# Twinklebear/tray_rust

Measured on NVIDIA H100. Metric: Mrays/s (primary+secondary), higher is better.
Workload: dtype f32

## Files before the change

tray_rust_b200/csrc/trb_api.cu:

```cuda
#include <chrono>
#include <dlfcn.h>
#include <nccl.h>
#include <cstdio>
#include <cstdlib>
#include <memory>
#include <thread>
#include <cub/device/device_radix_sort.cuh>
#include "trb_host.h"
#include "trb_kernels.cuh"

using namespace trbh;

namespace {

thread_local std::string g_error;
unsigned long long g_launches = 0;
trb_status fail(trb_status s, const std::string& msg) { g_error = msg; return s; }

#define CU(call)                                                                                                   \
    do {                                                                                                           \
        cudaError_t e_ = (call);                                                                                   \
        if (e_ != cudaSuccess) return fail(e_ == cudaErrorMemoryAllocation ? TRB_OOM : TRB_CUDA,                   \
                                           std::string(#call) + ": " + cudaGetErrorString(e_));                    \
    } while (0)
// ... 76 lines not shown
        for (int k = 0; k < 3; ++k) if (!(in[c].bmin[k] >= in[p].bmin[k] && in[c].bmax[k] <= in[p].bmax[k])) return false;
        return true;
    };
    if (in.empty()) { root_ref = QUAD_EMPTY_HOST; return true; }
    if (is_leaf(0)) { root_ref = leaf_ref(0); return ok; }
    std::vector<uint32_t> quad_of(in.size(), 0xffffffffu), order, todo{0};
    while (!todo.empty()) {
        const uint32_t p = todo.back(); todo.pop_back();
        quad_of[p] = (uint32_t)order.size(); order.push_back(p);
        uint32_t kids[4]; int nk = 0;
        for (uint32_t c : {p + 1, in[p].a}) {
            if (is_leaf(c)) continue;
            const uint32_t g0 = c + 1, g1 = in[c].a;
            if (inside(g0, c) && inside(g1, c)) { if (!is_leaf(g0)) kids[nk++] = g0; if (!is_leaf(g1)) kids[nk++] = g1; }
            else kids[nk++] = c;
        }
        for (int k = nk; k-- > 0;) todo.push_back(kids[k]);
    }
    if (order.size() >= (1u << 30)) return false;
    out.resize(order.size());
    auto slot = [&](trb::DQuad& q, int k, uint32_t node, bool empty) {
        if (empty) { q.q[2 * k] = make_float4(0.f, 0.f, 0.f, bits_f(0xffffffffu)); q.q[2 * k + 1] = make_float4(0.f, 0.f, 0.f, 0.f); return; }
        const uint32_t ref = is_leaf(node) ? leaf_ref(node) : (trb::REF_INTERIOR | quad_of[node]);
        q.q[2 * k] = make_float4(in[node].bmin[0], in[node].bmin[1], in[node].bmin[2], bits_f(ref));
        q.q[2 * k + 1] = make_float4(in[node].bmax[0], in[node].bmax[1], in[node].bmax[2], 0.f);
    };
    for (size_t qi = 0; qi < order.size(); ++qi) {
        const uint32_t p = order[qi];
        trb::DQuad& q = out[qi];
        uint32_t axes[2] = {0, 0};
        int h = 0;
        for (uint32_t c : {p + 1, in[p].a}) {
            bool split = false;
            if (!is_leaf(c)) { const uint32_t g0 = c + 1, g1 = in[c].a; split = inside(g0, c) && inside(g1, c); }
            if (split) { slot(q, 2 * h, c + 1, false); slot(q, 2 * h + 1, in[c].a, false); axes[h] = in[c].b & 3u; }
            else { slot(q, 2 * h, c, false); slot(q, 2 * h + 1, 0, true); }
            ++h;
        }
        q.q[1].w = bits_f((in[p].b & 3u) | axes[0] << 2 | axes[1] << 4);
    }
    root_ref = trb::REF_INTERIOR | quad_of[0];
    return ok;
}

}

namespace {
struct Tuning {
    int refill = 8;
    unsigned trace_grid = 0;
    uint32_t sched = 6;
    int quads = 0;
    int exact_box = 0;
    int pipe = 36;
    int film_v2 = 1;
    int sort = 0;
    int sort_bits = 5;
    int sort_min_round = 1;
    int shade_anim_occ = 4;
    int frame_device = 1;
    int anim_table = 2;
    int shade_split = -1;
    int shade_sort = 1;
    int shade_kind = 1;
    uint64_t pass_paths = 1ull << 24;
};
int env_int(const char* name, int dflt) { const char* v = getenv(name); return v ? (int)strtol(v, nullptr, 0) : dflt; }
void tuning_from_env(Tuning& t) {
    t.refill = env_int("TRB_REFILL", t.refill); t.trace_grid = (unsigned)env_int("TRB_TRACE_GRID", (int)t.trace_grid);
    t.sched = (uint32_t)env_int("TRB_TRACE_SCHED", (int)t.sched); t.quads = env_int("TRB_TRACE_QUADS", t.quads); t.pipe = env_int("TRB_TRACE_PIPE", t.pipe);
    t.film_v2 = env_int("TRB_FILM_V2", t.film_v2); t.sort = env_int("TRB_SORT", t.sort); t.sort_bits = env_int("TRB_SORT_BITS", t.sort_bits);
    t.sort_min_round = env_int("TRB_SORT_MIN_ROUND", t.sort_min_round); t.shade_split = env_int("TRB_SHADE_SPLIT", t.shade_split); t.anim_table = env_int("TRB_ANIM_TABLE", t.anim_table); t.frame_device = env_int("TRB_FRAME_DEVICE", t.frame_device);
    if (getenv("TRB_PASS_PATHS")) t.pass_paths = strtoull(getenv("TRB_PASS_PATHS"), nullptr, 0);
}

}

struct BlockList {
    uint32_t key[5];
    std::vector<uint32_t> host;
    uint2* dev = nullptr;
};

struct trb_scene {
    int device = 0;
    int sm_count = 0;
    Tuning tune;
    trb_film film{};
    trb_integrator integrator{};
    std::vector<trb_camera> cameras;
    std::vector<trb_instance> instances;
    std::vector<trb_spline> splines;
    std::vector<trb_keyframe> keyframes;
    std::vector<float> knots;
    std::vector<trb_color_key> color_keys;
    std::vector<float> fov_floats;
    std::vector<trb_material> materials;
    std::vector<HostMesh> meshes;
    uint32_t spp_pow2 = 1;
    uint32_t n_anim = 0;
    bool frame_set = false; uint32_t last_frame = 0; float last_start = 0, last_end = 0;
    uint32_t material_kinds = 0;
    bool mixed_materials = false;
    bool anim_emission = false;
    uint32_t* d_anim_instances = nullptr;
    int active_camera = -1;
    float shutter_open = 0, shutter_close = 0;
    std::vector<Xf> world;
    std::vector<trb_bvh_node> tlas_nodes;
    std::vector<uint32_t> tlas_order;
    float table[256];
    DeviceArena arena;
    trb::DScene ds{};
    trb::DInstance* d_instances = nullptr;
    trb::DPair* d_tlas = nullptr;
    trb::DQuad* d_tlas_quads = nullptr;
    trb::DBvh* d_tlas_hdr = nullptr;
    uint32_t* d_tlas_order = nullptr;
    size_t tlas_capacity = 0;
    trb_bvh_node* d_tlas_nodes = nullptr;
    float* d_bounds = nullptr;
    float* d_build_f = nullptr;
    uint32_t* d_build_u = nullptr;
    uint32_t* d_build_counts = nullptr;
    uint32_t tlas_n_nodes = 0;
    bool instances_static_uploaded = false, host_frame_stale = false;
    std::vector<BlockList> block_lists;
    uint32_t* d_counter = nullptr;
    int* d_error = nullptr;
    trb::DStats* d_stats = nullptr;
    float4* d_film = nullptr;
    float* h_film_staging = nullptr;
    cudaEvent_t ev0 = nullptr, ev1 = nullptr;
    bool frame_ready = false;
    trb::WfState wf{};
    size_t wf_capacity = 0;
    std::vector<void*> wf_allocs;
    std::vector<std::pair<cudaEvent_t, cudaEvent_t>> trace_events;
    std::vector<std::pair<cudaEvent_t, cudaEvent_t>> event_pool;
    uint4* d_ad_state = nullptr;
    uint2* d_ad_list[2] = {nullptr, nullptr};
    uint32_t* d_ad_index[2] = {nullptr, nullptr};
    uint32_t* d_ad_flags = nullptr;
    uint32_t* d_ad_count = nullptr;
    uint32_t* d_ad_spp = nullptr;
    void* d_film_scratch = nullptr;
    size_t film_scratch_bytes = 0;
    ~trb_scene() {
        for (void* p : {(void*)d_ad_state, (void*)d_ad_list[0], (void*)d_ad_list[1], (void*)d_ad_index[0], (void*)d_ad_index[1], (void*)d_ad_flags,
                        (void*)d_ad_count, (void*)d_ad_spp, d_film_scratch}) if (p) cudaFree(p);
        for (auto& b : block_lists) cudaFree(b.dev);
        for (void* p : wf_allocs) cudaFree(p);
        for (auto& e : trace_events) { cudaEventDestroy(e.first); cudaEventDestroy(e.second); }
        for (auto& e : event_pool) { cudaEventDestroy(e.first); cudaEventDestroy(e.second); }
        if (h_film_staging) cudaFreeHost(h_film_staging);
        if (ev0) cudaEventDestroy(ev0);
        if (ev1) cudaEventDestroy(ev1);
    }
};

namespace {

Box3 shape_bounds(const trb_scene& s, const trb_instance& in) {
    Box3 b;
    switch (in.shape) {
        case TRB_SHAPE_SPHERE: for (int i = 0; i < 3; ++i) { b.lo[i] = -in.p0; b.hi[i] = in.p0; } break;
        case TRB_SHAPE_DISK: b.lo[0] = b.lo[1] = -in.p0; b.hi[0] = b.hi[1] = in.p0; b.lo[2] = -0.1f; b.hi[2] = 0.1f; break;
        case TRB_SHAPE_RECT: { const float hw = in.p0 / 2.0f, hh = in.p1 / 2.0f; b.lo[0] = -hw; b.lo[1] = -hh; b.hi[0] = hw; b.hi[1] = hh; b.lo[2] = b.hi[2] = 0.0f; break; }
        case TRB_SHAPE_MESH: b = s.meshes[in.mesh].bounds; break;
        default: for (int i = 0; i < 3; ++i) b.lo[i] = b.hi[i] = 0.0f;
    }
    return b;
}

trb_status validate(const trb_scene_desc* d) {
    if (!d) return fail(TRB_INVALID_ARG, "null scene description");
    if (d->abi_version != TRB_ABI_VERSION) return fail(TRB_INVALID_ARG, "trb_scene_desc.abi_version mismatch");
    if (d->film.width == 0 || d->film.height == 0 || d->film.width % 8 || d->film.height % 8)
        return fail(TRB_INVALID_ARG, "Image not evenly divided by blocks of (8, 8)");
    if (d->film.frames == 0) return fail(TRB_INVALID_ARG, "film.frames must be >= 1");
    if (d->n_instances == 0) return fail(TRB_INVALID_ARG, "Aborting: the scene does not have any objects!");
    if (d->n_cameras == 0) return fail(TRB_INVALID_ARG, "Error: A camera is required!");
    if (d->integrator.type > TRB_INTEGRATOR_NORMALS_DEBUG) return fail(TRB_INVALID_ARG, "Unrecognized integrator type");
    if (d->integrator.type == TRB_INTEGRATOR_PATH && d->integrator.max_depth > 57u) return fail(TRB_UNSUPPORTED, "max_depth > 57");
    if (d->integrator.type == TRB_INTEGRATOR_WHITTED && d->integrator.max_depth > 24u) return fail(TRB_UNSUPPORTED, "whitted max_depth > 24 (device recursion stack)");
    if (!(d->film.filter_w > 0.0f && d->film.filter_h > 0.0f)) return fail(TRB_INVALID_ARG, "filter width/height must be positive");
    if (floorf(d->film.filter_w / 0.5f) > 8.0f || floorf(d->film.filter_h / 0.5f) > 8.0f) return fail(TRB_UNSUPPORTED, "filter wider than 4 pixels");
    bool light = false;
    for (uint32_t i = 0; i < d->n_instances; ++i) {
        const trb_instance& in = d->instances[i];
        if (in.kind > TRB_INST_EMITTER_POINT || in.shape > TRB_SHAPE_MESH) return fail(TRB_INVALID_ARG, "unknown instance kind/shape");
        if (in.kind != TRB_INST_EMITTER_POINT && in.shape == TRB_SHAPE_NONE) return fail(TRB_INVALID_ARG, "instance without geometry");
        if (in.kind == TRB_INST_EMITTER_AREA && in.shape == TRB_SHAPE_MESH)
            return fail(TRB_INVALID_ARG, "Geometry of type 'mesh' is not sampleable and can't be used for area light geometry");
        if (in.shape == TRB_SHAPE_MESH && in.mesh >= d->n_meshes) return fail(TRB_INVALID_ARG, "mesh index out of range");
        if (in.kind != TRB_INST_EMITTER_POINT && in.material >= d->n_materials) return fail(TRB_INVALID_ARG, "material index out of range");
        if ((uint64_t)in.spline_first + in.n_splines > d->n_splines) return fail(TRB_INVALID_ARG, "spline range out of bounds");
        if (in.kind != TRB_INST_RECEIVER) {
            light = true;
            if (in.n_emission == 0 || (uint64_t)in.emission_first + in.n_emission > d->n_color_keys) return fail(TRB_INVALID_ARG, "An emission color is required for emitters");
        }
    }
    for (uint32_t k = 0; k < d->n_splines; ++k) {
        const trb_spline& sp = d->splines[k];
        if (sp.n_ctrl == 0 || (uint64_t)sp.ctrl_first + sp.n_ctrl > d->n_keyframes) return fail(TRB_INVALID_ARG, "spline control points out of bounds");
        if (sp.n_ctrl > 1) {
            if ((uint64_t)sp.knot_first + sp.n_knots > d->n_knots) return fail(TRB_INVALID_ARG, "spline knots out of bounds");
            if (sp.n_ctrl <= sp.degree) return fail(TRB_INVALID_ARG, "Too few control points for curve");
            if ((uint64_t)sp.n_knots != (uint64_t)sp.n_ctrl + sp.degree + 1) return fail(TRB_INVALID_ARG, "Invalid B-spline: knots.len() != control_points.len() + degree + 1");
            if (sp.degree > (uint32_t)trbh::kMaxSplineDegree) return fail(TRB_UNSUPPORTED, "B-spline degree above 5");
            for (uint32_t i = 0; i < sp.n_knots; ++i) if (d->knots[sp.knot_first + i] != d->knots[sp.knot_first + i]) return fail(TRB_INVALID_ARG, "NaN knot in B-spline");
        }
    }
    if (!light) return fail(TRB_INVALID_ARG, "At least one light is required");
    for (uint32_t i = 0; i < d->n_cameras; ++i) {
        const trb_camera& c = d->cameras[i];
        if (c.n_fov_ctrl) {
            if ((uint64_t)c.fov_ctrl_first + c.n_fov_ctrl > d->n_fov_floats || (uint64_t)c.fov_knot_first + c.n_fov_knots > d->n_fov_floats) return fail(TRB_INVALID_ARG, "fov spline out of bounds");
            if (c.n_fov_ctrl <= c.fov_degree) return fail(TRB_INVALID_ARG, "Too few control points for curve");
            if ((uint64_t)c.n_fov_knots != (uint64_t)c.n_fov_ctrl + c.fov_degree + 1) return fail(TRB_INVALID_ARG, "Invalid B-spline: knots.len() != control_points.len() + degree + 1");
            for (uint32_t i = 0; i < c.n_fov_knots; ++i) if (d->fov_floats[c.fov_knot_first + i] != d->fov_floats[c.fov_knot_first + i]) return fail(TRB_INVALID_ARG, "NaN knot in B-spline");
            if (c.fov_degree > (uint32_t)trbh::kMaxSplineDegree) return fail(TRB_UNSUPPORTED, "B-spline degree above 5");
        }
        if ((uint64_t)c.spline_first + c.n_splines > d->n_splines) return fail(TRB_INVALID_ARG, "camera spline range out of bounds");
    }
    for (uint32_t i = 0; i < d->n_materials; ++i) {
        if (d->materials[i].type > TRB_MAT_MERL) return fail(TRB_INVALID_ARG, "unrecognized material type");
        if (d->materials[i].type == TRB_MAT_MERL && d->materials[i].merl >= d->n_merl) return fail(TRB_INVALID_ARG, "merl table index out of range");
        for (int k = 0; k < 4; ++k) if (d->materials[i].tex[k] > d->n_textures) return fail(TRB_INVALID_ARG, "texture index out of range");
    }
    uint64_t texels = 0;
    for (uint32_t i = 0; i < d->n_textures; ++i)
        if (d->textures[i].n_images == 0 || (uint64_t)d->textures[i].first_image + d->textures[i].n_images > d->n_images) return fail(TRB_INVALID_ARG, "texture image range out of bounds");
    for (uint32_t i = 0; i < d->n_images; ++i) {
        if (d->images[i].width == 0 || d->images[i].height == 0 || !d->images[i].rgba8) return fail(TRB_INVALID_ARG, "empty image");
        texels += (uint64_t)d->images[i].width * d->images[i].height;
    }
    if (texels >= (1ull << 32)) return fail(TRB_UNSUPPORTED, "more than 2^32 texels of image textures");
    for (uint32_t i = 0; i < d->n_meshes; ++i) {
        const trb_mesh& m = d->meshes[i];
        if (m.n_tris == 0 || m.n_verts == 0) return fail(TRB_INVALID_ARG, "empty mesh");
        if (!m.positions || !m.normals || !m.texcoords || !m.indices) return fail(TRB_INVALID_ARG, "Normals and texture coordinates are required!");
        for (size_t k = 0; k < 3 * (size_t)m.n_tris; ++k) if (m.indices[k] >= m.n_verts) return fail(TRB_INVALID_ARG, "mesh index out of range");
    }
    return TRB_OK;
}

trb_status ensure_blocks(trb_scene* s, const trb_render_cfg* cfg, const uint2** d_blocks, uint32_t* n_blocks) {
    if (cfg->shard_count > 1 && cfg->shard_index >= cfg->shard_count) return fail(TRB_INVALID_ARG, "shard_index must be < shard_count");
    const uint32_t key[5] = {cfg->block_start, cfg->block_count, cfg->shard_index, cfg->shard_count, cfg->shard_chunk};
    for (const BlockList& b : s->block_lists)
        if (std::memcmp(b.key, key, sizeof key) == 0) { *d_blocks = b.dev; *n_blocks = (uint32_t)(b.host.size() / 2); return TRB_OK; }
    if (s->block_lists.size() >= 16) {
        CU(cudaDeviceSynchronize());
        for (BlockList& b : s->block_lists) cudaFree(b.dev);
        s->block_lists.clear();
    }
    BlockList bl;
    std::memcpy(bl.key, key, sizeof key);
    bl.host = morton_blocks(s->film.width, s->film.height, cfg->block_start, cfg->block_count, cfg->shard_index, cfg->shard_count, cfg->shard_chunk);
    const size_t n = bl.host.size() / 2;
    CU(cudaMalloc(reinterpret_cast<void**>(&bl.dev), std::max<size_t>(1, n) * sizeof(uint2)));
    if (n) { cudaError_t e = cudaMemcpy(bl.dev, bl.host.data(), n * sizeof(uint2), cudaMemcpyHostToDevice); if (e != cudaSuccess) { cudaFree(bl.dev); CU(e); } }
    s->block_lists.push_back(std::move(bl));
    *d_blocks = s->block_lists.back().dev; *n_blocks = (uint32_t)n;
    return TRB_OK;
}

trb_status resolve_samples(const trb_scene* s, const trb_render_cfg* cfg, uint32_t& spp, uint32_t& first, uint32_t& count) {
    if (cfg->spp > (1u << 31)) return fail(TRB_INVALID_ARG, "spp too large");
    spp = cfg->spp ? pow2_ceil(cfg->spp) : s->spp_pow2;
    first = cfg->sample_first;
    if (first > spp) return fail(TRB_INVALID_ARG, "sample_first exceeds spp");
    count = cfg->sample_count ? cfg->sample_count : spp - first;
    if ((uint64_t)first + count > spp) return fail(TRB_INVALID_ARG, "sample range exceeds spp");
    return TRB_OK;
}

template <bool STATS, int MODE, bool ANIM>
trb_status launch_render_t(trb_scene* s, const trb::RenderParams& rp, uint32_t flags, cudaStream_t st) {
    const int T = 9 + 2 * std::max(s->ds.fpw_x, s->ds.fpw_y);
    const size_t smem = (size_t)T * T * sizeof(float4);
    int per_sm = 0;
    CU(cudaOccupancyMaxActiveBlocksPerMultiprocessor(&per_sm, trb::k_render<STATS, MODE, ANIM>, trb::RENDER_THREADS, smem));
    const uint32_t grid = std::max(1u, std::min<uint32_t>(rp.n_blocks, (uint32_t)(std::max(1, per_sm) * s->sm_count)));
    trb::k_render<STATS, MODE, ANIM><<<grid, trb::RENDER_THREADS, smem, st>>>(s->ds, rp, flags);
    g_launches++;
    CU(cudaGetLastError());
    return TRB_OK;
}
trb_status ensure_wavefront(trb_scene* s, size_t n_paths) {
    if (n_paths <= s->wf_capacity) return TRB_OK;
    CU(cudaDeviceSynchronize());
    for (void* p : s->wf_allocs) cudaFree(p);
    s->wf_allocs.clear(); s->wf_capacity = 0;
    const size_t cap = n_paths;
    cudaError_t err = cudaSuccess;
    auto grab = [&](size_t bytes, void** out) {
        if (err != cudaSuccess) return;
        err = cudaMalloc(out, bytes);
        if (err == cudaSuccess) s->wf_allocs.push_back(*out);
    };
    trb::WfState& w = s->wf;
    float4** f4[] = {&w.org, &w.cont, &w.shadow, &w.mis, &w.a, &w.b, &w.tprev, &w.thr, &w.illum, &w.ng, &w.rad, &w.f_p, &w.f_n, &w.f_t, &w.f_b};
    for (float4** q : f4) grab(cap * sizeof(float4), reinterpret_cast<void**>(q));
    grab(cap * sizeof(uint4), reinterpret_cast<void**>(&w.hit));
    uint32_t** u1[] = {&w.q_active[0], &w.q_active[1], &w.q_ending[0], &w.q_ending[1], &w.q_cont, &w.q_shadow, &w.q_mis};
    for (uint32_t** q : u1) grab(cap * sizeof(uint32_t), reinterpret_cast<void**>(q));
    grab(cap * trb::WF_MID_BUCKETS * sizeof(uint32_t), reinterpret_cast<void**>(&w.q_mid));
    grab(64 * trb::WF_CNT * sizeof(uint32_t), reinterpret_cast<void**>(&w.counters));
    const size_t max_bins = (size_t)3 * (8u << (3 * trb::WF_SORT_MAX_BITS));
    uint32_t** u3[] = {&w.q_sorted, &w.sort_key, &w.sort_rank};
    for (uint32_t** q : u3) grab(3 * cap * sizeof(uint32_t), reinterpret_cast<void**>(q));
    grab(max_bins * sizeof(uint32_t), reinterpret_cast<void**>(&w.sort_hist));
    grab(max_bins * sizeof(uint32_t), reinterpret_cast<void**>(&w.sort_offs));
    grab(64 * 8 * sizeof(uint32_t), reinterpret_cast<void**>(&w.bounds));
    w.xf_tab = nullptr; w.n_anim = s->n_anim;
    if (s->n_anim) grab(cap * (size_t)s->n_anim * 32 * sizeof(float), reinterpret_cast<void**>(&w.xf_tab));
    if (err == cudaSuccess) err = cudaMemset(w.sort_hist, 0, max_bins * sizeof(uint32_t));
    if (err != cudaSuccess) {
        for (void* p : s->wf_allocs) cudaFree(p);
        s->wf_allocs.clear();
        cudaGetLastError();
        return fail(err == cudaErrorMemoryAllocation ? TRB_OOM : TRB_CUDA, std::string("wavefront state: ") + cudaGetErrorString(err));
    }
    s->wf_capacity = cap;
    return TRB_OK;
}

void launch_anim_table(trb_scene* s, trb::WfState& wf, size_t n_paths, bool adapt, cudaStream_t st) {
    if (!(s->ds.has_anim && wf.xf_tab && s->tune.anim_table)) { wf.xf_tab = nullptr; return; }
    const size_t items = n_paths * wf.n_anim;
    const uint32_t nu = s->ds.n_uniq_splines;
    if (s->tune.anim_table >= 2 && nu > 0 && nu <= 256) {
        const uint32_t per_iter = std::max(1u, std::min(32u, 128u / nu));
        const size_t smem = (size_t)per_iter * nu * 32 * sizeof(float);
        const unsigned grid = (unsigned)std::min<size_t>((n_paths + per_iter - 1) / per_iter, (size_t)s->sm_count * 16);
        if (adapt) trb::k_wf_anim_table2<true><<<grid, 128, smem, st>>>(s->ds, wf, per_iter);
        else trb::k_wf_anim_table2<<<grid, 128, smem, st>>>(s->ds, wf, per_iter);
    } else {
        const unsigned grid = (unsigned)std::min<size_t>((items + 127) / 128, (size_t)s->sm_count * 16);
        if (adapt) trb::k_wf_anim_table<true><<<grid, 128, 0, st>>>(s->ds, wf);
        else trb::k_wf_anim_table<<<grid, 128, 0, st>>>(s->ds, wf);
    }
    g_launches++;
}

void launch_query_trace(trb_scene* s, const trb::RenderParams& rp, const trb::WfState& wf, uint32_t tflags, bool stats, const uint32_t* q_sorted,
                        cudaStream_t st) {
    const Tuning& tu = s->tune;
    const bool anim = s->ds.has_anim != 0;
    const unsigned resident = stats ? 4u : (anim ? 8u : 9u);
    const unsigned tgrid = (unsigned)s->sm_count * (tu.trace_grid ? tu.trace_grid : 2u * resident);
    const uint32_t sched = std::max(1u, tu.sched);
    if (anim) {
        if (stats) trb::k_wf_trace<true, 4, 16, true, true, false, 97><<<tgrid, 128, 0, st>>>(s->ds, rp, wf, 0, tflags, tu.refill, sched, q_sorted);
        else trb::k_wf_trace<false, 8, 12, true, true, false, 97><<<tgrid, 128, 0, st>>>(s->ds, rp, wf, 0, tflags, tu.refill, sched, q_sorted);
    } else if (stats) trb::k_wf_trace<true, 4, 16, false, true, false, 97><<<tgrid, 128, 0, st>>>(s->ds, rp, wf, 0, tflags, tu.refill, sched, q_sorted);
    else trb::k_wf_trace<false, 9, 12, false, true, false, 97><<<tgrid, 128, 0, st>>>(s->ds, rp, wf, 0, tflags, tu.refill, sched, q_sorted);
}

template <int MODE>
void launch_shade(trb_scene* s, const trb::RenderParams& rp, const trb::WfState& wf, uint32_t round, cudaStream_t st) {
    const Tuning& tu = s->tune;
    const bool anim = s->ds.has_anim != 0;
    const unsigned shade_grid = (unsigned)s->sm_count * 4;
    constexpr int MB = MODE == 2 ? 2 : 0;
    const bool split_auto = s->mixed_materials || (tu.shade_sort && tu.shade_kind && s->material_kinds == (1u << TRB_MAT_MATTE));
    if (tu.shade_split > 0 || (tu.shade_split < 0 && split_auto)) {
        const uint32_t all = 0xffu, own = (tu.shade_sort && tu.shade_kind) ? (s->material_kinds & (1u << TRB_MAT_MATTE)) : 0u;
        const uint32_t rest = tu.shade_sort ? (s->material_kinds & ~own) : all;
        if (anim) {
            trb::k_wf_shade_a<MODE, true, 3><<<shade_grid, 128, 0, st>>>(s->ds, rp, wf, round);
            if (own) trb::k_wf_shade_b<true, 4, TRB_MAT_MATTE, MB><<<shade_grid, 128, 0, st>>>(s->ds, rp, wf, round, own);
            if (rest) trb::k_wf_shade_b<true, 3, -1, MB><<<shade_grid, 128, 0, st>>>(s->ds, rp, wf, round, rest);
            if (own) trb::k_wf_shade_c<MODE, true, 6, TRB_MAT_MATTE><<<(unsigned)s->sm_count * 6, 128, 0, st>>>(s->ds, rp, wf, round, own);
            if (rest) trb::k_wf_shade_c<MODE, true, 4><<<shade_grid, 128, 0, st>>>(s->ds, rp, wf, round, rest);
        } else {
            const unsigned ga = (unsigned)s->sm_count * 6, gb = (unsigned)s->sm_count * 5, gc = (unsigned)s->sm_count * 6;
            trb::k_wf_shade_a<MODE, false, 6><<<ga, 128, 0, st>>>(s->ds, rp, wf, round);
            if (own) trb::k_wf_shade_b<false, 5, TRB_MAT_MATTE, MB><<<gb, 128, 0, st>>>(s->ds, rp, wf, round, own);
            if (rest) trb::k_wf_shade_b<false, 5, -1, MB><<<gb, 128, 0, st>>>(s->ds, rp, wf, round, rest);
            if (own) trb::k_wf_shade_c<MODE, false, 6, TRB_MAT_MATTE><<<gc, 128, 0, st>>>(s->ds, rp, wf, round, own);
            if (rest) trb::k_wf_shade_c<MODE, false, 6><<<gc, 128, 0, st>>>(s->ds, rp, wf, round, rest);
        }
        g_launches += 4;
        return;
    }
    if (anim) {
        if constexpr (MODE == 1) trb::k_wf_shade<1, true, 3><<<shade_grid, 128, 0, st>>>(s->ds, rp, wf, round);
        else if constexpr (MODE == 2) trb::k_wf_shade<2, true, 4><<<shade_grid, 128, 0, st>>>(s->ds, rp, wf, round);
        else if (tu.shade_anim_occ >= 4) trb::k_wf_shade<0, true, 4><<<shade_grid, 128, 0, st>>>(s->ds, rp, wf, round);
        else trb::k_wf_shade<0, true, 3><<<shade_grid, 128, 0, st>>>(s->ds, rp, wf, round);
    } else trb::k_wf_shade<MODE, false, 4><<<shade_grid, 128, 0, st>>>(s->ds, rp, wf, round);
    g_launches += 2;
}

trb_status wavefront_rounds(trb_scene* s, const trb::RenderParams& rp, const trb::WfState& wf, uint32_t flags, int mode, cudaStream_t st) {
    const Tuning& tu = s->tune;
    const bool stats = (flags & TRB_RENDER_STATS) != 0, anim = s->ds.has_anim != 0;
    const uint32_t rounds = s->integrator.max_depth + 2;
    const int refill = tu.refill;
    const unsigned resident = (flags & TRB_RENDER_STATS) ? 4u : (tu.pipe == 0 || tu.pipe == 1 || tu.pipe == 33 ? 7u : (tu.pipe == 34 || tu.pipe == 35 || s->ds.has_anim ? 8u : 9u));
    const unsigned tgrid = (unsigned)s->sm_count * (tu.trace_grid ? tu.trace_grid : 2u * resident);
    const uint32_t sched = tu.sched;
    const bool quads = tu.quads != 0;
    const uint32_t tflags = flags | (tu.exact_box ? trb::WF_TRACE_FORCE_EXACT_BOX : 0u);
    for (uint32_t round = 0; round < rounds; ++round) {
        const uint32_t* q_sorted = nullptr;
        if (tu.sort && (int)round >= tu.sort_min_round) {
            const uint32_t bits = (uint32_t)std::min(trb::WF_SORT_MAX_BITS, std::max(1, tu.sort_bits));
            const unsigned sgrid = (unsigned)s->sm_count * 8;
            trb::k_wf_sort_count<<<sgrid, 256, 0, st>>>(wf, round, bits, tu.sort == 2 ? 1u : 0u);
            trb::k_wf_sort_scan<<<1, 1024, 0, st>>>(wf, 3u * (8u << (3u * bits)));
            trb::k_wf_sort_scatter<<<sgrid, 256, 0, st>>>(wf, round);
            g_launches += 3;
            q_sorted = wf.q_sorted;
        }
        std::pair<cudaEvent_t, cudaEvent_t> ev{nullptr, nullptr};
        if (flags & TRB_RENDER_TIME_TRACE) {
            if (!s->event_pool.empty()) { ev = s->event_pool.back(); s->event_pool.pop_back(); }
            else { CU(cudaEventCreate(&ev.first)); CU(cudaEventCreate(&ev.second)); }
            CU(cudaEventRecord(ev.first, st));
        }
#define TRB_TRACE_LAUNCH(ST, MB, SS, AN, PH, QD, PIPE) trb::k_wf_trace<ST, MB, SS, AN, PH, QD, PIPE><<<tgrid, 128, 0, st>>>(s->ds, rp, wf, round, tflags, refill, sched, q_sorted)
        const bool v2 = tu.pipe != 0;
        if (mode == 2 && round == 0) launch_query_trace(s, rp, wf, tflags, stats, q_sorted, st);
        else if (anim) {
            if (stats) { if (v2) TRB_TRACE_LAUNCH(true, 4, 16, true, true, false, 33); else TRB_TRACE_LAUNCH(true, 4, 16, true, true, false, 0); }
            else if (!v2) TRB_TRACE_LAUNCH(false, 7, 16, true, true, false, 0);
            else if (tu.pipe == 33) TRB_TRACE_LAUNCH(false, 7, 16, true, true, false, 33);
            else if (tu.pipe == 37) TRB_TRACE_LAUNCH(false, 9, 12, true, true, false, 33);
            else TRB_TRACE_LAUNCH(false, 8, 12, true, true, false, 33);
        } else if (stats) {
            if (sched == 0) TRB_TRACE_LAUNCH(true, 4, 16, false, false, false, 0);
            else if (v2) TRB_TRACE_LAUNCH(true, 4, 16, false, true, false, 33); else TRB_TRACE_LAUNCH(true, 4, 16, false, true, false, 0);
        } else if (sched == 0) TRB_TRACE_LAUNCH(false, 7, 16, false, false, false, 0);
        else if (quads) TRB_TRACE_LAUNCH(false, 7, 16, false, true, true, 0);
        else switch (tu.pipe) {
            case 0: TRB_TRACE_LAUNCH(false, 7, 16, false, true, false, 0); break;
            case 1: TRB_TRACE_LAUNCH(false, 7, 16, false, true, false, 1); break;
            case 33: TRB_TRACE_LAUNCH(false, 7, 16, false, true, false, 33); break;
            case 34: TRB_TRACE_LAUNCH(false, 8, 16, false, true, false, 33); break;
            case 35: TRB_TRACE_LAUNCH(false, 8, 12, false, true, false, 33); break;
            case 37: TRB_TRACE_LAUNCH(false, 9, 8, false, true, false, 33); break;
            default: TRB_TRACE_LAUNCH(false, 9, 12, false, true, false, 33); break;
        }
#undef TRB_TRACE_LAUNCH
        if (ev.first) { CU(cudaEventRecord(ev.second, st)); s->trace_events.push_back(ev); }
        if (mode == 0) launch_shade<0>(s, rp, wf, round, st);
        else if (mode == 1) launch_shade<1>(s, rp, wf, round, st);
        else launch_shade<2>(s, rp, wf, round, st);
    }
    CU(cudaGetLastError());
    return TRB_OK;
}

trb_status launch_wavefront(trb_scene* s, const trb::RenderParams& rp, uint32_t flags, int mode, cudaStream_t st) {
    const size_t n_paths = (size_t)rp.n_blocks * 64 * rp.sample_count;
    if (n_paths > s->wf_capacity || n_paths >= (1ull << 30)) return fail(TRB_INVALID_ARG, "pass larger than the wavefront state");
    const Tuning& tu = s->tune;
    trb::WfState wf = s->wf;
    wf.n_paths = (uint32_t)n_paths;
    wf.mid_keyed = s->tune.shade_sort ? 1u : 0u;
    if (s->integrator.type != TRB_INTEGRATOR_PATH) {
        const unsigned grid = (unsigned)std::min<size_t>((n_paths + 127) / 128, (size_t)s->sm_count * 8);
        const bool anim = s->ds.has_anim != 0;
        if (anim) { if (mode == 0) trb::k_simple_integrator<0, true><<<grid, 128, 0, st>>>(s->ds, rp, wf.rad, wf.n_paths, s->integrator.type, flags, nullptr);
                    else trb::k_simple_integrator<1, true><<<grid, 128, 0, st>>>(s->ds, rp, wf.rad, wf.n_paths, s->integrator.type, flags, nullptr); }
        else if (mode == 0) trb::k_simple_integrator<0, false><<<grid, 128, 0, st>>>(s->ds, rp, wf.rad, wf.n_paths, s->integrator.type, flags, nullptr);
        else trb::k_simple_integrator<1, false><<<grid, 128, 0, st>>>(s->ds, rp, wf.rad, wf.n_paths, s->integrator.type, flags, nullptr);
        g_launches++;
        if (mode == 0) {
            const int T = 9 + 2 * std::max(s->ds.fpw_x, s->ds.fpw_y);
            const unsigned film_grid = std::min<unsigned>(rp.n_blocks, (unsigned)s->sm_count * 8);
            if (tu.film_v2) trb::k_wf_film_v2<<<film_grid, trb::RENDER_THREADS, (size_t)4 * T * T * sizeof(float4), st>>>(s->ds, rp, wf);
            else trb::k_wf_film<<<film_grid, trb::RENDER_THREADS, (size_t)T * T * sizeof(float4), st>>>(s->ds, rp, wf);
            g_launches++;
        }
        CU(cudaGetLastError());
        return TRB_OK;
    }
    CU(cudaMemsetAsync(wf.counters, 0, 64 * trb::WF_CNT * sizeof(uint32_t), st));
    const unsigned gen_grid = (unsigned)std::min<size_t>((n_paths + 255) / 256, (size_t)s->sm_count * 8);
    const bool anim = s->ds.has_anim != 0;
    if (rp.ad_state) {
        if (anim) trb::k_wf_generate_ad<true><<<gen_grid, 256, 0, st>>>(s->ds, rp, wf);
        else trb::k_wf_generate_ad<false><<<gen_grid, 256, 0, st>>>(s->ds, rp, wf);
    } else if (anim) trb::k_wf_generate<true><<<gen_grid, 256, 0, st>>>(s->ds, rp, wf);
    else trb::k_wf_generate<false><<<gen_grid, 256, 0, st>>>(s->ds, rp, wf);
    g_launches++;
    launch_anim_table(s, wf, n_paths, rp.ad_state != nullptr, st);
    const trb_status r = wavefront_rounds(s, rp, wf, flags, mode, st);
    if (r != TRB_OK) return r;
    if (mode == 0 && rp.film) {
        const int T = 9 + 2 * std::max(s->ds.fpw_x, s->ds.fpw_y);
        const unsigned film_grid = std::min<unsigned>(rp.n_blocks, (unsigned)s->sm_count * 8);
        if (rp.ad_state) {
            if (tu.film_v2) trb::k_wf_film_v2<true><<<film_grid, trb::RENDER_THREADS, (size_t)4 * T * T * sizeof(float4), st>>>(s->ds, rp, wf);
            else trb::k_wf_film<true><<<film_grid, trb::RENDER_THREADS, (size_t)T * T * sizeof(float4), st>>>(s->ds, rp, wf);
        } else if (tu.film_v2) trb::k_wf_film_v2<<<film_grid, trb::RENDER_THREADS, (size_t)4 * T * T * sizeof(float4), st>>>(s->ds, rp, wf);
        else trb::k_wf_film<<<film_grid, trb::RENDER_THREADS, (size_t)T * T * sizeof(float4), st>>>(s->ds, rp, wf);
        g_launches++;
    }
    CU(cudaGetLastError());
    return TRB_OK;
}

trb_status render_passes(trb_scene* s, trb::RenderParams rp, uint32_t flags, int mode, cudaStream_t st) {
    const uint32_t nb = rp.n_blocks, first = rp.sample_first, count = rp.sample_count;
    const uint2* blocks = rp.blocks;
    const uint64_t total = (uint64_t)nb * 64 * count;
    uint64_t want = std::min<uint64_t>(total, std::min<uint64_t>(std::max<uint64_t>(s->tune.pass_paths, 64), (1ull << 30) - 64));
    if (mode == 1) {
        if (total >= (1ull << 30)) return fail(TRB_INVALID_ARG, "sample buffer too large: blocks*64*sample_count must be < 2^30; select fewer blocks or samples");
        want = total;
    }
    want = ((want + 63) / 64) * 64;
    if (want > s->wf_capacity) {
        trb_status r;
        while ((r = ensure_wavefront(s, (size_t)want)) == TRB_OOM && want > (1u << 16) && mode == 0) want = ((want / 2 + 63) / 64) * 64;
        if (r != TRB_OK) return r;
    }
    const uint64_t cap = std::max<uint64_t>(want, 64);
    uint32_t bp, sp;
    if ((uint64_t)nb * 64 <= cap) { bp = nb; sp = (uint32_t)std::min<uint64_t>(count, cap / ((uint64_t)nb * 64)); }
    else { bp = (uint32_t)(cap / 64); sp = 1; }
    for (uint32_t b0 = 0; b0 < nb; b0 += bp)
        for (uint32_t s0 = 0; s0 < count; s0 += sp) {
            rp.blocks = blocks + b0; rp.n_blocks = std::min(bp, nb - b0);
            rp.sample_first = first + s0; rp.sample_count = std::min(sp, count - s0);
            trb_status r = launch_wavefront(s, rp, flags, mode, st);
            if (r != TRB_OK) return r;
        }
    return TRB_OK;
}

trb_status adaptive_check(const trb_scene* s, const trb_render_cfg* cfg, const trb_adaptive* ad, trbh::AdSchedule& sch) {
    if (cfg->spp || cfg->sample_first || cfg->sample_count)
        return fail(TRB_INVALID_ARG, "the Adaptive sampler owns the sample schedule: spp, sample_first and sample_count must be 0");
    if (!trbh::ad_schedule(ad->min_spp, ad->max_spp, sch))
        return fail(TRB_INVALID_ARG, "Adaptive sampler: max_spp < min_spp after rounding up to powers of two (the reference panics), or more than 2^24");
    if (s->integrator.type != TRB_INTEGRATOR_PATH) return fail(TRB_UNSUPPORTED, "the Adaptive sampler is built for the path integrator only");
    if (cfg->flags & TRB_RENDER_MEGAKERNEL) return fail(TRB_UNSUPPORTED, "the Adaptive sampler runs on the wavefront pipeline only");
    return TRB_OK;
}

trb_status ensure_adaptive(trb_scene* s) {
    if (s->d_ad_state) return TRB_OK;
    const size_t npx = (size_t)s->film.width * s->film.height, nblk = npx / 64;
    CU(cudaMalloc(reinterpret_cast<void**>(&s->d_ad_state), npx * sizeof(uint4)));
    for (int k = 0; k < 2; ++k) {
        CU(cudaMalloc(reinterpret_cast<void**>(&s->d_ad_list[k]), std::max<size_t>(1, nblk) * sizeof(uint2)));
        CU(cudaMalloc(reinterpret_cast<void**>(&s->d_ad_index[k]), std::max<size_t>(1, nblk) * sizeof(uint32_t)));
    }
    CU(cudaMalloc(reinterpret_cast<void**>(&s->d_ad_flags), std::max<size_t>(1, nblk) * sizeof(uint32_t)));
    CU(cudaMemset(s->d_ad_flags, 0, std::max<size_t>(1, nblk) * sizeof(uint32_t)));
    CU(cudaMalloc(reinterpret_cast<void**>(&s->d_ad_count), 2 * sizeof(uint32_t)));
    CU(cudaMalloc(reinterpret_cast<void**>(&s->d_ad_spp), npx * sizeof(uint32_t)));
    return TRB_OK;
}

trb_status render_adaptive_rounds(trb_scene* s, const trbh::AdSchedule& sch, trb::RenderParams rp, const uint2* d_blocks, uint32_t nb, uint32_t flags,
                                  cudaStream_t st, uint32_t* d_spp) {
    trb_status r = ensure_adaptive(s);
    if (r != TRB_OK) return r;
    const uint64_t per_block = (uint64_t)64 * std::max(sch.min, sch.step);
    if (per_block >= (1ull << 30)) return fail(TRB_INVALID_ARG, "Adaptive sampler: one block of one round exceeds 2^30 paths");
    uint64_t want = std::min<uint64_t>((uint64_t)nb * per_block, std::min<uint64_t>(std::max<uint64_t>(s->tune.pass_paths, 64), (1ull << 30) - 64));
    want = ((std::max(want, per_block) + 63) / 64) * 64;
    if (want > s->wf_capacity) {
        while ((r = ensure_wavefront(s, (size_t)want)) == TRB_OOM && want / 2 >= per_block && want > (1u << 16)) want = ((want / 2 + 63) / 64) * 64;
        if (r != TRB_OK) return r;
    }
    const uint64_t cap = want;
    rp.ad_state = s->d_ad_state;
    rp.ad_min = sch.min; rp.ad_max = sch.max; rp.ad_step = sch.step; rp.ad_max_per_pixel = sch.max_per_pixel;
    rp.spp = sch.max; rp.ad_time_len = sch.max;
    const unsigned init_grid = (unsigned)std::min<size_t>(((size_t)nb * 64 + 255) / 256, (size_t)s->sm_count * 8);
    trb::k_ad_init<<<std::max(1u, init_grid), 256, 0, st>>>(s->ds, d_blocks, nb, s->d_ad_state, s->d_ad_list[0], s->d_ad_index[0], s->d_ad_count);
    g_launches++;
    for (uint32_t round = 0; round < sch.rounds; ++round) {
        const int cur = round & 1;
        const uint32_t count = trbh::ad_count(sch, round);
        rp.ad_round = round; rp.sample_first = trbh::ad_slot_base(sch, round); rp.sample_count = count;
        rp.ld_offset = trbh::ad_offset(sch, round); rp.ad_pos_len = count;
        rp.ad_live = s->d_ad_count + cur;
        const uint32_t bp = (uint32_t)std::max<uint64_t>(1, cap / ((uint64_t)64 * count));
        for (uint32_t b0 = 0; b0 < nb; b0 += bp) {
            rp.blocks = s->d_ad_list[cur] + b0; rp.n_blocks = std::min(bp, nb - b0); rp.ad_block_index = s->d_ad_index[cur] + b0; rp.ad_b0 = b0;
            r = launch_wavefront(s, rp, flags, 0, st);
            if (r != TRB_OK) return r;
            const unsigned dgrid = (unsigned)std::min<size_t>(((size_t)rp.n_blocks * 64 + 127) / 128, (size_t)s->sm_count * 16);
            trb::k_ad_decide<<<dgrid, 128, 0, st>>>(s->ds, rp, s->wf, s->d_ad_flags + b0);
            g_launches++;
        }
        if (round + 1 == sch.rounds) break;
        trb::k_ad_compact<<<1, 1024, 0, st>>>(s->d_ad_flags, s->d_ad_count + cur, s->d_ad_list[cur], s->d_ad_index[cur], s->d_ad_list[cur ^ 1],
                                              s->d_ad_index[cur ^ 1], s->d_ad_count + (cur ^ 1));
        g_launches++;
    }
    if (d_spp) {
        const unsigned sgrid = (unsigned)std::min<size_t>(((size_t)nb * 64 + 255) / 256, (size_t)s->sm_count * 8);
        trb::k_ad_pixel_spp<<<std::max(1u, sgrid), 256, 0, st>>>(s->ds, d_blocks, nb, s->d_ad_state, d_spp);
        g_launches++;
    }
    CU(cudaGetLastError());
    return TRB_OK;
// ... 1739 lines not shown
```

tray_rust_b200/csrc/trb_kernels.cuh:

```cuda
#pragma once
#include "trb_device.h"
#include "trb_detmath.cuh"
#include "trb_anim.h"
#include "trb_adaptive.h"
#include "../../include/trb.h"

namespace trb {

struct f3 { float x, y, z; };
TRB_HD __forceinline__ f3 mk(float x, float y, float z) { f3 r; r.x = x; r.y = y; r.z = z; return r; }
__device__ __forceinline__ f3 splat(float v) { return mk(v, v, v); }
__device__ __forceinline__ f3 operator+(f3 a, f3 b) { return mk(a.x + b.x, a.y + b.y, a.z + b.z); }
__device__ __forceinline__ f3 operator-(f3 a, f3 b) { return mk(a.x - b.x, a.y - b.y, a.z - b.z); }
__device__ __forceinline__ f3 operator*(f3 a, f3 b) { return mk(a.x * b.x, a.y * b.y, a.z * b.z); }
__device__ __forceinline__ float ieee_div(float a, float b) { return a / b; }
__device__ __forceinline__ float ieee_sqrt(float a) { return sqrtf(a); }
__device__ __forceinline__ f3 operator/(f3 a, f3 b) { return mk(ieee_div(a.x, b.x), ieee_div(a.y, b.y), ieee_div(a.z, b.z)); }
__device__ __forceinline__ f3 operator*(f3 a, float s) { return mk(a.x * s, a.y * s, a.z * s); }
__device__ __forceinline__ f3 operator*(float s, f3 a) { return mk(s * a.x, s * a.y, s * a.z); }
__device__ __forceinline__ f3 operator/(f3 a, float s) { return mk(ieee_div(a.x, s), ieee_div(a.y, s), ieee_div(a.z, s)); }
__device__ __forceinline__ f3 operator-(f3 a) { return mk(-a.x, -a.y, -a.z); }
__device__ __forceinline__ float dot3(f3 a, f3 b) { return a.x * b.x + a.y * b.y + a.z * b.z; }
__device__ __forceinline__ f3 cross3(f3 a, f3 b) { return mk(a.y * b.z - a.z * b.y, a.z * b.x - a.x * b.z, a.x * b.y - a.y * b.x); }
__device__ __forceinline__ float len2(f3 a) { return a.x * a.x + a.y * a.y + a.z * a.z; }
// ... 1248 lines not shown
            if (delta) ds.a = f * lrad * fabsf(dot3(wi, fr.n)) / pdf_light;
            else {
                const float pdf_bsdf = bsdf_pdf<KIND>(m, fr, wo, wi, BX_NON_SPECULAR);
                const float w = power_heuristic(pdf_light, pdf_bsdf);
                ds.a = f * lrad * fabsf(dot3(wi, fr.n)) * w / pdf_light;
            }
        }
    }
    if (!delta) {
        f3 f, wi2; float pdf_bsdf; uint32_t sampled;
        bsdf_sample<KIND>(sc, m, fr, wo, BX_NON_SPECULAR, b0, b1, bc, f, wi2, pdf_bsdf, sampled);
        if (pdf_bsdf > 0.0f && !black(f)) {
            float w = 1.0f;
            bool go = true;
            if (!(sampled & BX_SPECULAR)) {
                const f3 pl = xf_point(linv, p);
                const f3 wl = unit(xf_vector(linv, wi2));
                const float pl_pdf = shape_pdf(shape, p0, p1, pl, wl);
                if (pl_pdf == 0.0f) go = false;
                else w = power_heuristic(pdf_bsdf, pl_pdf);
            }
            if (go) {
                ds.has_mis = true; ds.mis_d = wi2;
                ds.b = f * emission * fabsf(dot3(wi2, fr.n)) * w / pdf_bsdf;
            }
        }
    }
}
template <bool ANIM>
__device__ __forceinline__ bool mis_sees_light(const DScene& sc, f3 org, f3 mis_d, uint32_t li, uint32_t hit_inst, float hit_t, float time, const float* xf_row = nullptr) {
    if (hit_inst != li) return false;
    const DInstance& light = sc.instances[li];
    f3 le;
    emission_at<ANIM>(sc, light, time, le.x, le.y, le.z);
    if (black(le)) return false;
    Ray mr; mr.o = org; mr.d = mis_d; mr.tmin = 0.001f; mr.tmax = hit_t;
    HitRec mh; mh.t = hit_t; mh.inst = hit_inst; mh.prim = 0; mh.b1 = 0.0f; mh.b2 = 0.0f;
    Surf s;
    surface_at<ANIM>(sc, mr, mh, s, time, xf_row);
    return dot3(-mis_d, s.ng) > 0.0f;
}
__device__ __forceinline__ f3 direct_resolve(f3 a, f3 b, bool occluded, bool mis_ok) {
    f3 direct = occluded ? splat(0.0f) : a;
    if (mis_ok) direct = direct + b;
    return direct;
}

struct BounceOut {
    DirectSetup ds;
    uint32_t light;
    f3 t_before;
    f3 throughput;
    f3 next_d;
    f3 org;
    bool specular, terminate;
};
template <bool ANIM>
__device__ __forceinline__ void bounce_emission(const DScene& sc, uint32_t hit_inst, f3 ray_d, f3 first_ng, uint32_t bounce, bool prev_specular, f3 throughput_in,
                                                float time, f3& illum) {
    const DInstance& in = sc.instances[hit_inst];
    if (bounce == 0 || prev_specular) {
        if (__ldg(&in.kind) != TRB_INST_RECEIVER) {
            const f3 w = -ray_d;
            if (dot3(w, first_ng) > 0.0f) {
                f3 le;
                emission_at<ANIM>(sc, in, time, le.x, le.y, le.z);
                illum = illum + throughput_in * le;
            }
        }
    }
}
template <bool ANIM, int KIND = -1>
__device__ __forceinline__ void bounce_direct(const DScene& sc, const Mat& m, const Frame& fr, f3 wo, uint32_t bounce, uint32_t hsample, float time, DirectSetup& ds,
                                              uint32_t& light, const float* xf_row = nullptr, uint32_t ld_off = 0) {
    PathRng rng; rng.h = hsample; rng.len = sc.max_depth + 1; rng.off = ld_off;
    float l0, l1, b0, b1;
    rng.two_d(bounce, S_L0, S_L1, S_L_PERM, l0, l1);
    rng.two_d(bounce, S_B0, S_B1, S_B_PERM, b0, b1);
    const float lc = rng.one_d(bounce, S_LC, S_LC_PERM), bc = rng.one_d(bounce, S_BC, S_BC_PERM);
    uint32_t l = f2u(lc * (float)sc.n_lights);
    if (l > sc.n_lights - 1) l = sc.n_lights - 1;
    light = __ldg(&sc.lights[l]);
    direct_setup<ANIM, KIND>(sc, m, fr, wo, light, l0, l1, b0, b1, bc, time, ds, xf_row);
}
struct ScatterOut { f3 throughput, next_d; bool specular, terminate; };
template <int KIND = -1>
__device__ __forceinline__ void bounce_scatter(const DScene& sc, const Mat& m, const Frame& fr, f3 wo, uint32_t bounce, uint32_t hsample, f3 throughput_in, ScatterOut& o, uint32_t ld_off = 0) {
    PathRng rng; rng.h = hsample; rng.len = sc.max_depth + 1; rng.off = ld_off;
    float q0, q1;
    rng.two_d(bounce, S_P0, S_P1, S_P_PERM, q0, q1);
    const float qc = rng.one_d(bounce, S_PC, S_PC_PERM);
    f3 f, wi; float pdf; uint32_t sampled;
    bsdf_sample<KIND>(sc, m, fr, wo, BX_ALL, q0, q1, qc, f, wi, pdf, sampled);
    o.throughput = throughput_in; o.next_d = splat(0.0f); o.specular = false; o.terminate = true;
    if (black(f) || pdf == 0.0f) return;
    o.specular = (sampled & BX_SPECULAR) != 0;
    f3 t = throughput_in * f * fabsf(dot3(wi, fr.n)) / pdf;
    if (bounce > sc.min_depth) {
        const float lum = 0.2126f * t.x + 0.7152f * t.y + 0.0722f * t.z;
        const float cont = fmaxf(0.5f, lum);
        if (unit_f32(rng.draw(S_RR + bounce)) > cont) { o.throughput = t; return; }
        t = t / cont;
    }
    o.throughput = t;
    if (bounce == sc.max_depth) return;
    o.next_d = unit(wi);
    o.terminate = false;
}
template <bool ANIM>
__device__ __forceinline__ void shade_bounce(const DScene& sc, const Surf& s, uint32_t hit_inst, f3 ray_d, f3 first_ng, uint32_t bounce, bool prev_specular,
                                             uint32_t hsample, f3 throughput_in, float time, f3& illum, BounceOut& o, const float* xf_row = nullptr,
                                             uint32_t ld_off = 0) {
    bounce_emission<ANIM>(sc, hit_inst, ray_d, first_ng, bounce, prev_specular, throughput_in, time, illum);
    Mat m;
    load_mat_at(sc, __ldg(&sc.instances[hit_inst].material), s.u, s.v, time, m);
    Frame fr;
    make_frame(s, fr);
    const f3 wo = -ray_d;
    bounce_direct<ANIM>(sc, m, fr, wo, bounce, hsample, time, o.ds, o.light, xf_row, ld_off);
    o.t_before = throughput_in;
    o.org = fr.p;
    ScatterOut so;
    bounce_scatter(sc, m, fr, wo, bounce, hsample, throughput_in, so, ld_off);
    o.throughput = so.throughput; o.next_d = so.next_d; o.specular = so.specular; o.terminate = so.terminate;
}

template <bool ANIM>
__device__ __forceinline__ float camera_ray(const DScene& sc, float sx, float sy, float tm, Ray& ray) {
    const f3 pc = xf_point(sc.cam.px_to_cam, mk(sx, sy, 0.0f));
    const f3 pp = mk(sc.cam.scaling[0], sc.cam.scaling[1], sc.cam.scaling[2]) * pc;
    const f3 d = unit(pp);
    const float frame_time = (sc.cam.shutter_close - sc.cam.shutter_open) * tm + sc.cam.shutter_open;
    if (ANIM && sc.cam.animated) {
        float inv[16], mat[16];
        eval_anim_xf(sc, sc.cam.spline_first, sc.cam.n_splines, frame_time, inv, mat);
        ray.o = xf_point(mat, splat(0.0f));
        ray.d = xf_vector(mat, d);
    } else {
        ray.o = xf_point(sc.cam.cam_mat, splat(0.0f));
        ray.d = xf_vector(sc.cam.cam_mat, d);
    }
    ray.tmin = 0.0f; ray.tmax = finf();
    return frame_time;
}

template <bool STATS, bool ANIM>
__device__ f3 radiance_of_sample(const DScene& sc, Ray ray, float time, uint32_t hpix_sample, bool ref_shadow, RayCounts& rc, Cnt& cnt, int* err) {
    HitRec hit;
    rc.primary++;
    if (!scene_trace<STATS, ANIM>(sc, ray, hit, false, cnt, err, time)) return splat(0.0f);
    f3 illum = splat(0.0f), throughput = splat(1.0f);
    bool specular_bounce = false;
    uint32_t bounce = 0;
    Surf s;
    surface_at<ANIM>(sc, ray, hit, s, time);
    const f3 first_ng = s.ng;
    for (;;) {
        BounceOut o;
        shade_bounce<ANIM>(sc, s, hit.inst, ray.d, first_ng, bounce, specular_bounce, hpix_sample, throughput, time, illum, o);
        bool occluded = false, mis_ok = false;
        if (o.ds.has_shadow) {
            Ray sr; sr.o = o.org; sr.d = o.ds.shadow_d; sr.tmin = 0.001f; sr.tmax = 0.999f;
            HitRec sh;
            rc.shadow++;
            occluded = scene_trace<STATS, ANIM>(sc, sr, sh, !ref_shadow, cnt, err, time);
        }
        if (o.ds.has_mis) {
            Ray mr; mr.o = o.org; mr.d = o.ds.mis_d; mr.tmin = 0.001f; mr.tmax = finf();
            HitRec mh;
            rc.mis++;
            if (scene_trace<STATS, ANIM>(sc, mr, mh, false, cnt, err, time)) mis_ok = mis_sees_light<ANIM>(sc, o.org, o.ds.mis_d, o.light, mh.inst, mh.t, time);
        }
        illum = illum + o.t_before * direct_resolve(o.ds.a, o.ds.b, occluded, mis_ok);
        throughput = o.throughput;
        specular_bounce = o.specular;
        if (o.terminate) break;
        ray.o = o.org; ray.d = o.next_d; ray.tmin = 0.001f; ray.tmax = finf();
        rc.cont++;
        if (!scene_trace<STATS, ANIM>(sc, ray, hit, false, cnt, err, time)) break;
        surface_at<ANIM>(sc, ray, hit, s, time);
        bounce += 1;
    }
    return illum;
}

struct PixelStreams { uint32_t scr0, scr1, kpos, scrt, ktime, hpix; };
__device__ __forceinline__ PixelStreams pixel_streams(uint32_t seed, uint32_t pixel) {
    PixelStreams p;
    p.hpix = rng_absorb(rng_seed(seed), pixel);
    const uint32_t hs = rng_absorb(p.hpix, PIXEL_STREAM);
    p.scr0 = scramble_of(rng_absorb(hs, PX_POS0));
    p.scr1 = scramble_of(rng_absorb(hs, PX_POS1));
    p.kpos = rng_absorb(hs, PX_POS_PERM);
    p.scrt = scramble_of(rng_absorb(hs, PX_TIME));
    p.ktime = rng_absorb(hs, PX_TIME_PERM);
    return p;
}

__device__ __forceinline__ void flush_stats(DStats* st, const RayCounts& rc, const Cnt& cnt, uint32_t samples, bool with_tests) {
    unsigned long long v[8] = {samples, rc.primary, rc.shadow, rc.mis, rc.cont, cnt.node, cnt.tri, cnt.inst};
    const int n = with_tests ? 8 : 5;
    for (int i = 0; i < n; ++i) {
        unsigned long long x = v[i];
        for (int o = 16; o > 0; o >>= 1) x += __shfl_xor_sync(0xffffffffu, x, o);
        if ((threadIdx.x & 31) == 0 && x) atomicAdd(&reinterpret_cast<unsigned long long*>(st)[i], x);
    }
}

__device__ __forceinline__ bool lock_block_takes(float s, int i, int lo, int hi, int fpw) {
    const int b0 = (i >> 1) << 1;
    const int w0 = max(lo, b0), w1 = min(hi + 1, b0 + 2);
    return s >= (float)(w0 - fpw) && s < (float)(w1 + fpw);
}

__device__ __forceinline__ void splat_sample(const DScene& sc, float4* tile, const float* s_table, int T, int tx0, int ty0, int x_lo, int x_hi, int y_lo,
                                             int y_hi, uint32_t px, uint32_t py, float sx, float sy, f3 c) {
    const float img_x = sx - 0.5f, img_y = sy - 0.5f;
    const int ry = (int)ceilf(sc.filter_h / sc.filter_inv_h) + 1, rx = (int)ceilf(sc.filter_w / sc.filter_inv_w) + 1;
    const int iy0 = max(y_lo, (int)py - ry), iy1 = min(y_hi, (int)py + ry + 1);
    const int ix0 = max(x_lo, (int)px - rx), ix1 = min(x_hi, (int)px + rx + 1);
    for (int iy = iy0; iy <= iy1; ++iy) {
        const float fy = fabsf((float)iy - img_y) * sc.filter_inv_h;
        if (fy > sc.filter_h) continue;
        if (sc.film_block_filter && !lock_block_takes(sy, iy, y_lo, y_hi, sc.fpw_y)) continue;
        const uint32_t fyi = min(f2u(fy * 16.0f), 15u);
        for (int ix = ix0; ix <= ix1; ++ix) {
            const float fx = fabsf((float)ix - img_x) * sc.filter_inv_w;
            if (fx > sc.filter_w) continue;
            if (sc.film_block_filter && !lock_block_takes(sx, ix, x_lo, x_hi, sc.fpw_x)) continue;
            const uint32_t fxi = min(f2u(fx * 16.0f), 15u);
            const float wgt = s_table[fyi * 16 + fxi];
            float* t = reinterpret_cast<float*>(&tile[(iy - ty0) * T + (ix - tx0)]);
            atomicAdd(t + 0, wgt * c.x);
            atomicAdd(t + 1, wgt * c.y);
            atomicAdd(t + 2, wgt * c.z);
            atomicAdd(t + 3, wgt);
        }
    }
}

constexpr int RENDER_THREADS = 128;
constexpr int MAX_TILE = 25;

template <bool STATS, int MODE, bool ANIM>
__global__ void __launch_bounds__(RENDER_THREADS) k_render(const __grid_constant__ DScene sc, const __grid_constant__ RenderParams rp, uint32_t flags) {
    extern __shared__ float4 tile[];
    __shared__ float s_table[256];
    __shared__ uint32_t s_item;
    const int T = 9 + 2 * max(sc.fpw_x, sc.fpw_y);
    const bool ref_shadow = (flags & 4u) != 0;
    for (int i = threadIdx.x; i < 256; i += RENDER_THREADS) s_table[i] = sc.filter_table[i];
    RayCounts rc = {0, 0, 0, 0};
    Cnt cnt = {0, 0, 0};
    uint32_t my_samples = 0;
    const uint32_t pix = threadIdx.x & 63, lane_s = threadIdx.x >> 6;
    for (;;) {
        __syncthreads();
        if (threadIdx.x == 0) s_item = atomicAdd(rp.work_counter, 1u);
        if (MODE == 0) for (int i = threadIdx.x; i < T * T; i += RENDER_THREADS) tile[i] = make_float4(0.f, 0.f, 0.f, 0.f);
        __syncthreads();
        const uint32_t item = s_item;
        if (item >= rp.n_blocks) break;
        const uint2 blk = rp.blocks[item];
        const uint32_t bx = blk.x * 8, by = blk.y * 8;
        const uint32_t px = bx + (pix & 7), py = by + (pix >> 3);
        const uint32_t pixel = py * sc.width + px;
        const PixelStreams ps = pixel_streams(rp.seed, pixel);
        const int x_lo = max((int)bx - sc.fpw_x, 0), x_hi = min((int)bx + 8 + sc.fpw_x, (int)sc.width - 1);
        const int y_lo = max((int)by - sc.fpw_y, 0), y_hi = min((int)by + 8 + sc.fpw_y, (int)sc.height - 1);
        const int tx0 = (int)bx - sc.fpw_x, ty0 = (int)by - sc.fpw_y;
        for (uint32_t si = rp.sample_first + lane_s; si < rp.sample_first + rp.sample_count; si += 2) {
            const uint32_t ip = permute_index(si, rp.spp, ps.kpos);
            const float sx = ld_vdc(ip, ps.scr0) + (float)px;
            const float sy = ld_sobol(ip, ps.scr1) + (float)py;
            const float tm = ld_vdc(permute_index(si, rp.spp, ps.ktime), ps.scrt);
            Ray ray;
            const float time = camera_ray<ANIM>(sc, sx, sy, tm, ray);
            my_samples++;
            f3 c = radiance_of_sample<STATS, ANIM>(sc, ray, time, rng_absorb(ps.hpix, si), ref_shadow, rc, cnt, rp.error_flag);
            c = mk(clampf(c.x, 0.0f, 1.0f), clampf(c.y, 0.0f, 1.0f), clampf(c.z, 0.0f, 1.0f));
            if (MODE == 1) {
                trb_sample* out = reinterpret_cast<trb_sample*>(rp.samples_out) + ((size_t)item * 64 + pix) * rp.sample_count + (si - rp.sample_first);
                out->x = sx; out->y = sy; out->r = c.x; out->g = c.y; out->b = c.z;
            } else {
                splat_sample(sc, tile, s_table, T, tx0, ty0, x_lo, x_hi, y_lo, y_hi, px, py, sx, sy, c);
            }
        }
        if (MODE == 0) {
            __syncthreads();
            for (int i = threadIdx.x; i < T * T; i += RENDER_THREADS) {
                const int ix = tx0 + i % T, iy = ty0 + i / T;
                if (ix < x_lo || ix > x_hi || iy < y_lo || iy > y_hi) continue;
                const float4 v = tile[i];
                if (v.w == 0.0f && v.x == 0.0f && v.y == 0.0f && v.z == 0.0f) continue;
                float* dst = reinterpret_cast<float*>(rp.film + (size_t)iy * sc.width + ix);
                atomicAdd(dst + 0, v.x); atomicAdd(dst + 1, v.y); atomicAdd(dst + 2, v.z); atomicAdd(dst + 3, v.w);
            }
        }
    }
    if (rp.stats) flush_stats(rp.stats, rc, cnt, my_samples, STATS);
}

struct WfState {
    float4* org;
    float4* cont;
    uint4* hit;
    float4* shadow;
    float4* mis;
    float4* a;
    float4* b;
    float4* tprev;
    float4* thr;
    float4* illum;
    float4* ng;
    float4* rad;
    uint32_t* q_active[2];
    uint32_t* q_ending[2];
    uint32_t* q_cont; uint32_t* q_shadow; uint32_t* q_mis;
    uint32_t* counters;
    uint32_t n_paths;
    uint32_t* q_sorted;
    uint32_t* sort_key;
    uint32_t* sort_rank;
    uint32_t* sort_hist;
    uint32_t* sort_offs;
    float4* f_p;
    float4* f_n;
    float4* f_t;
    float4* f_b;
    uint32_t* q_mid;
    uint32_t mid_keyed;
    float* xf_tab;
    uint32_t n_anim;
    uint32_t* bounds;
};
constexpr uint32_t WF_PATH_MASK = 0x3fffffffu;
constexpr int WF_SORT_MAX_BITS = 6;
enum { WF_N_ACTIVE = 0, WF_N_CONT = 1, WF_N_SHADOW = 2, WF_N_MIS = 3, WF_TRACE_HEAD = 4, WF_SHADE_HEAD = 5, WF_N_MID = 6, WF_SHADE_B_HEAD = 7, WF_SHADE_C_HEAD = 8,
       WF_N_ENDING = 9, WF_ENDING_HEAD = 10,
       WF_N_PATHS = 11,
       WF_MID_K = 12, WF_B_HEAD_K = 20, WF_C_HEAD_K = 28, WF_CNT = 36 };
constexpr uint32_t WF_MID_BUCKETS = 8;
enum { WF_F_SPECULAR = 1u, WF_F_TERMINATE = 2u, WF_F_SHADOW = 4u, WF_F_MIS = 8u };

struct SampleId { uint32_t item, pix, si, px, py, pixel; };
__device__ __forceinline__ SampleId sample_id(const DScene& sc, const RenderParams& rp, uint32_t p) {
    SampleId id;
    const uint32_t s = p % rp.sample_count, q = p / rp.sample_count;
    id.pix = q & 63; id.item = q >> 6; id.si = rp.sample_first + s;
    const uint2 blk = rp.blocks[id.item];
    id.px = blk.x * 8 + (id.pix & 7); id.py = blk.y * 8 + (id.pix >> 3);
    id.pixel = id.py * sc.width + id.px;
    return id;
}
__device__ __forceinline__ void sample_position(const RenderParams& rp, const PixelStreams& ps, const SampleId& id, float& sx, float& sy, float& tm) {
    const uint32_t ip = permute_index(id.si, rp.spp, ps.kpos);
    sx = ld_vdc(ip, ps.scr0) + (float)id.px;
    sy = ld_sobol(ip, ps.scr1) + (float)id.py;
    tm = ld_vdc(permute_index(id.si, rp.spp, ps.ktime), ps.scrt);
}
__device__ __forceinline__ PixelStreams pixel_streams_round(uint32_t seed, uint32_t pixel, uint32_t round) {
    PixelStreams p;
    p.hpix = rng_absorb(rng_seed(seed), pixel);
    const uint32_t hs = rng_absorb(p.hpix, AD_PIXEL_STREAM0 - round);
    p.scr0 = scramble_of(rng_absorb(hs, PX_POS0));
    p.scr1 = scramble_of(rng_absorb(hs, PX_POS1));
    p.kpos = rng_absorb(hs, PX_POS_PERM);
    p.scrt = scramble_of(rng_absorb(hs, PX_TIME));
    p.ktime = rng_absorb(hs, PX_TIME_PERM);
    return p;
}
__device__ __forceinline__ void sample_position_ad(const RenderParams& rp, const PixelStreams& ps, const SampleId& id, float& sx, float& sy, float& tm) {
    const uint32_t s = id.si - rp.sample_first;
    const uint32_t ip = permute_index(s, rp.ad_pos_len, ps.kpos) + rp.ld_offset;
    sx = ld_vdc(ip, ps.scr0) + (float)id.px;
    sy = ld_sobol(ip, ps.scr1) + (float)id.py;
    tm = ld_vdc(permute_index(s, rp.ad_time_len, ps.ktime) + rp.ld_offset, ps.scrt);
}
__device__ __forceinline__ uint32_t ad_pass_blocks(const RenderParams& rp) {
    const uint32_t live = *rp.ad_live;
    return live > rp.ad_b0 ? min(rp.n_blocks, live - rp.ad_b0) : 0u;
}

__device__ __forceinline__ void wf_push(uint32_t* q, uint32_t* counter, bool want, uint32_t value) {
    const unsigned mask = __ballot_sync(0xffffffffu, want);
    if (mask == 0) return;
    const int lane = threadIdx.x & 31, leader = __ffs(mask) - 1;
    uint32_t base = 0;
    if (lane == leader) base = atomicAdd(counter, (uint32_t)__popc(mask));
    base = __shfl_sync(0xffffffffu, base, leader);
    if (want) q[base + __popc(mask & ((1u << lane) - 1u))] = value;
}

__device__ __forceinline__ void wf_push_keyed(uint32_t* q, uint32_t stride, uint32_t* counters, bool want, uint32_t key, uint32_t value) {
    const unsigned mask = __ballot_sync(0xffffffffu, want);
    if (mask == 0 || !want) return;
    const unsigned peers = __match_any_sync(mask, key);
    const int lane = threadIdx.x & 31, leader = __ffs(peers) - 1;
    uint32_t base = 0;
    if (lane == leader) base = atomicAdd(&counters[key], (uint32_t)__popc(peers));
    base = __shfl_sync(peers, base, leader);
    q[(size_t)key * stride + base + __popc(peers & ((1u << lane) - 1u))] = value;
}

template <bool ANIM>
__device__ __forceinline__ const float* wf_xf_row(const WfState& wf, uint32_t p) {
    return (ANIM && wf.xf_tab) ? wf.xf_tab + (size_t)p * wf.n_anim * 32 : nullptr;
}
template <bool ADAPT = false>
__global__ void __launch_bounds__(128) k_wf_anim_table(const __grid_constant__ DScene sc, const __grid_constant__ WfState wf) {
    const size_t n = (size_t)(ADAPT ? wf.counters[WF_N_PATHS] : wf.n_paths) * wf.n_anim;
    for (size_t i = blockIdx.x * (size_t)blockDim.x + threadIdx.x; i < n; i += (size_t)gridDim.x * blockDim.x) {
        const uint32_t p = (uint32_t)(i / wf.n_anim), k = (uint32_t)(i % wf.n_anim);
        const DInstance& in = sc.instances[__ldg(&sc.anim_instances[k])];
        float inv[16], mat[16];
        eval_anim_xf(sc, __ldg(&in.spline_first), __ldg(&in.n_splines), wf.thr[p].w, inv, mat);
        float4* dst = reinterpret_cast<float4*>(wf.xf_tab + i * 32);
#pragma unroll
        for (int q = 0; q < 4; ++q) dst[q] = make_float4(inv[4 * q], inv[4 * q + 1], inv[4 * q + 2], inv[4 * q + 3]);
#pragma unroll
        for (int q = 0; q < 4; ++q) dst[4 + q] = make_float4(mat[4 * q], mat[4 * q + 1], mat[4 * q + 2], mat[4 * q + 3]);
    }
}

template <bool ADAPT = false>
__global__ void __launch_bounds__(128) k_wf_anim_table2(const __grid_constant__ DScene sc, const __grid_constant__ WfState wf, uint32_t per_iter) {
    extern __shared__ float s_lvl[];
    const uint32_t nu = sc.n_uniq_splines;
    const uint32_t n_paths = ADAPT ? wf.counters[WF_N_PATHS] : wf.n_paths;
    for (uint32_t p0 = blockIdx.x * per_iter; p0 < n_paths; p0 += gridDim.x * per_iter) {
        const uint32_t np = min(per_iter, n_paths - p0);
        for (uint32_t i = threadIdx.x; i < np * nu; i += blockDim.x) {
            const uint32_t lp = i / nu, u = i % nu;
            const trb_spline& sp = sc.splines[__ldg(&sc.uniq_splines[u])];
            const float time = wf.thr[p0 + lp].w;
            const float lo = sc.knots[sp.knot_first + sp.degree], hi = sc.knots[sp.knot_first + sp.n_knots - 1 - sp.degree];
            const trbh::Xf t = trbh::keyframe_xf(trbh::spline_point(sp, sc.keyframes, sc.knots, trbh::clampf_hd(time, lo, hi)));
            float* dst = s_lvl + (size_t)i * 32;
#pragma unroll
            for (int q = 0; q < 16; ++q) { dst[q] = t.fwd.m[q]; dst[16 + q] = t.inv.m[q]; }
        }
        __syncthreads();
        for (uint32_t i = threadIdx.x; i < np * wf.n_anim; i += blockDim.x) {
            const uint32_t lp = i / wf.n_anim, k = i % wf.n_anim;
            const DInstance& in = sc.instances[__ldg(&sc.anim_instances[k])];
            const uint32_t first = __ldg(&in.spline_first), count = __ldg(&in.n_splines);
            trbh::Xf acc = trbh::xf_identity();
            for (uint32_t s = first; s < first + count; ++s) {
                trbh::Xf t;
                if (sc.splines[s].n_ctrl == 1) t = sc.level_xf[s];
                else {
                    const float* src = s_lvl + ((size_t)lp * nu + __ldg(&sc.spline_uniq[s])) * 32;
#pragma unroll
                    for (int q = 0; q < 16; ++q) { t.fwd.m[q] = src[q]; t.inv.m[q] = src[16 + q]; }
                }
                acc = trbh::xf_compose(t, acc);
            }
            float4* dst = reinterpret_cast<float4*>(wf.xf_tab + ((size_t)(p0 + lp) * wf.n_anim + k) * 32);
#pragma unroll
            for (int q = 0; q < 4; ++q) dst[q] = make_float4(acc.inv.m[4 * q], acc.inv.m[4 * q + 1], acc.inv.m[4 * q + 2], acc.inv.m[4 * q + 3]);
#pragma unroll
            for (int q = 0; q < 4; ++q) dst[4 + q] = make_float4(acc.fwd.m[4 * q], acc.fwd.m[4 * q + 1], acc.fwd.m[4 * q + 2], acc.fwd.m[4 * q + 3]);
        }
        __syncthreads();
    }
}

__device__ __forceinline__ uint32_t f_ordered(float f) { const uint32_t u = __float_as_uint(f); return (u & 0x80000000u) ? ~u : (u | 0x80000000u); }
__device__ __forceinline__ float f_unordered(uint32_t u) { return __uint_as_float((u & 0x80000000u) ? (u & 0x7fffffffu) : ~u); }
__device__ __forceinline__ void wf_bounds_add(uint32_t* b, bool have, f3 o) {
    float lx = have ? o.x : finf(), ly = have ? o.y : finf(), lz = have ? o.z : finf();
    float hx = have ? o.x : -finf(), hy = have ? o.y : -finf(), hz = have ? o.z : -finf();
    if (__ballot_sync(0xffffffffu, have) == 0) return;
#pragma unroll
    for (int s = 16; s > 0; s >>= 1) {
        lx = fminf(lx, __shfl_xor_sync(0xffffffffu, lx, s)); ly = fminf(ly, __shfl_xor_sync(0xffffffffu, ly, s)); lz = fminf(lz, __shfl_xor_sync(0xffffffffu, lz, s));
        hx = fmaxf(hx, __shfl_xor_sync(0xffffffffu, hx, s)); hy = fmaxf(hy, __shfl_xor_sync(0xffffffffu, hy, s)); hz = fmaxf(hz, __shfl_xor_sync(0xffffffffu, hz, s));
    }
    if ((threadIdx.x & 31) == 0) {
        atomicMin(b + 0, f_ordered(lx)); atomicMin(b + 1, f_ordered(ly)); atomicMin(b + 2, f_ordered(lz));
        atomicMax(b + 4, f_ordered(hx)); atomicMax(b + 5, f_ordered(hy)); atomicMax(b + 6, f_ordered(hz));
    }
}

__device__ __forceinline__ uint32_t spread3(uint32_t x) {
    x &= 0x3ffu; x = (x | (x << 16)) & 0x030000ffu; x = (x | (x << 8)) & 0x0300f00fu; x = (x | (x << 4)) & 0x030c30c3u; x = (x | (x << 2)) & 0x09249249u;
    return x;
}
struct RayRef { uint32_t type, p; };
__device__ __forceinline__ RayRef wf_ray_ref(const WfState& wf, uint32_t i, uint32_t n_cont, uint32_t n_shadow) {
    RayRef r;
    if (i < n_cont) { r.type = 0; r.p = wf.q_cont[i]; }
    else if (i < n_cont + n_shadow) { r.type = 1; r.p = wf.q_shadow[i - n_cont]; }
    else { r.type = 2; r.p = wf.q_mis[i - n_cont - n_shadow]; }
    return r;
}
__global__ void __launch_bounds__(256) k_wf_sort_count(const __grid_constant__ WfState wf, uint32_t round, uint32_t bits, uint32_t cell_major) {
    const uint32_t* cnt_r = wf.counters + round * WF_CNT;
    const uint32_t n_cont = cnt_r[WF_N_CONT], n_shadow = cnt_r[WF_N_SHADOW], total = n_cont + n_shadow + cnt_r[WF_N_MIS];
    const uint32_t* b = wf.bounds + round * 8;
    const f3 lo = mk(f_unordered(b[0]), f_unordered(b[1]), f_unordered(b[2])), hi = mk(f_unordered(b[4]), f_unordered(b[5]), f_unordered(b[6]));
    const float cells = (float)(1u << bits);
    const float sx = hi.x > lo.x ? cells / (hi.x - lo.x) : 0.0f, sy = hi.y > lo.y ? cells / (hi.y - lo.y) : 0.0f, sz = hi.z > lo.z ? cells / (hi.z - lo.z) : 0.0f;
    const uint32_t cmax = (1u << bits) - 1u, nb = 8u << (3u * bits);
    for (uint32_t i = blockIdx.x * blockDim.x + threadIdx.x; i < total; i += gridDim.x * blockDim.x) {
        const RayRef r = wf_ray_ref(wf, i, n_cont, n_shadow);
        const float4 o4 = wf.org[r.p];
        const float4 d4 = r.type == 0 ? wf.cont[r.p] : (r.type == 1 ? wf.shadow[r.p] : wf.mis[r.p]);
        const uint32_t cx = min(cmax, __float2uint_rz(fmaxf(0.0f, (o4.x - lo.x) * sx))), cy = min(cmax, __float2uint_rz(fmaxf(0.0f, (o4.y - lo.y) * sy))),
                       cz = min(cmax, __float2uint_rz(fmaxf(0.0f, (o4.z - lo.z) * sz)));
        const uint32_t m = spread3(cx) | (spread3(cy) << 1) | (spread3(cz) << 2);
        const uint32_t oct = (d4.x < 0.0f ? 1u : 0u) | (d4.y < 0.0f ? 2u : 0u) | (d4.z < 0.0f ? 4u : 0u);
        const uint32_t key = r.type * nb + (cell_major ? ((m << 3) | oct) : ((oct << (3u * bits)) | m));
        wf.sort_key[i] = key;
        wf.sort_rank[i] = atomicAdd(&wf.sort_hist[key], 1u);
    }
}
__global__ void __launch_bounds__(1024) k_wf_sort_scan(const __grid_constant__ WfState wf, uint32_t n_bins) {
    __shared__ uint32_t part[1024];
    const uint32_t chunk = (n_bins + 1023u) / 1024u, b0 = min(n_bins, threadIdx.x * chunk), b1 = min(n_bins, b0 + chunk);
    uint32_t sum = 0;
    for (uint32_t k = b0; k < b1; ++k) sum += wf.sort_hist[k];
    part[threadIdx.x] = sum;
    __syncthreads();
    for (uint32_t s = 1; s < 1024; s <<= 1) {
        const uint32_t v = threadIdx.x >= s ? part[threadIdx.x - s] : 0u;
        __syncthreads();
        part[threadIdx.x] += v;
        __syncthreads();
    }
    uint32_t run = part[threadIdx.x] - sum;
    for (uint32_t k = b0; k < b1; ++k) { const uint32_t c = wf.sort_hist[k]; wf.sort_offs[k] = run; wf.sort_hist[k] = 0u; run += c; }
}
__global__ void __launch_bounds__(256) k_wf_sort_scatter(const __grid_constant__ WfState wf, uint32_t round) {
    const uint32_t* cnt_r = wf.counters + round * WF_CNT;
    const uint32_t n_cont = cnt_r[WF_N_CONT], n_shadow = cnt_r[WF_N_SHADOW], total = n_cont + n_shadow + cnt_r[WF_N_MIS];
    for (uint32_t i = blockIdx.x * blockDim.x + threadIdx.x; i < total; i += gridDim.x * blockDim.x) {
        const RayRef r = wf_ray_ref(wf, i, n_cont, n_shadow);
        wf.q_sorted[wf.sort_offs[wf.sort_key[i]] + wf.sort_rank[i]] = (r.type << 30) | r.p;
    }
}

template <bool ANIM>
__global__ void __launch_bounds__(256) k_wf_generate(const __grid_constant__ DScene sc, const __grid_constant__ RenderParams rp, const __grid_constant__ WfState wf) {
    const uint32_t n = wf.n_paths;
    for (uint32_t p = blockIdx.x * blockDim.x + threadIdx.x; p < n; p += gridDim.x * blockDim.x) {
        const SampleId id = sample_id(sc, rp, p);
        const PixelStreams ps = pixel_streams(rp.seed, id.pixel);
        float sx, sy, tm;
        sample_position(rp, ps, id, sx, sy, tm);
        Ray ray;
        const float time = camera_ray<ANIM>(sc, sx, sy, tm, ray);
        wf.org[p] = make_float4(ray.o.x, ray.o.y, ray.o.z, __uint_as_float(0u));
        wf.cont[p] = make_float4(ray.d.x, ray.d.y, ray.d.z, finf());
        wf.thr[p] = make_float4(1.0f, 1.0f, 1.0f, time);
        wf.illum[p] = make_float4(0.0f, 0.0f, 0.0f, 0.0f);
        wf.q_cont[p] = p;
    }
    if (blockIdx.x == 0 && threadIdx.x == 0) {
        wf.counters[WF_N_ACTIVE] = n; wf.counters[WF_N_CONT] = n;
        if (rp.stats) { atomicAdd(&rp.stats->camera_samples, (unsigned long long)n); }
    }
    if (blockIdx.x == 0 && threadIdx.x < 64) {
        uint32_t* b = wf.bounds + threadIdx.x * 8;
        b[0] = b[1] = b[2] = b[3] = 0xffffffffu; b[4] = b[5] = b[6] = b[7] = 0u;
    }
}

template <bool STATS, int MINB, int SMEM_STACK, bool ANIM, bool PHASED, bool QUADS, int PIPE = 0>
__global__ void __launch_bounds__(128, MINB) k_wf_trace(const __grid_constant__ DScene sc, const __grid_constant__ RenderParams rp, const __grid_constant__ WfState wf,
                                                         uint32_t round, uint32_t flags, int WF_REFILL_IDLE, uint32_t sched, const uint32_t* __restrict__ q_sorted) {
    constexpr bool HOME = PHASED && (PIPE & 32) != 0;
    constexpr bool QUERY = (PIPE & 64) != 0;
    uint32_t* cnt_r = wf.counters + round * WF_CNT;
    const uint32_t n_cont = cnt_r[WF_N_CONT], n_shadow = cnt_r[WF_N_SHADOW], n_mis = cnt_r[WF_N_MIS];
    const uint32_t total = n_cont + n_shadow + n_mis;
    const bool shadow_any = (flags & 4u) == 0;
    const int lane = threadIdx.x & 31;
    const unsigned lt_mask = (1u << lane) - 1u;
    Cnt cnt = {0, 0, 0};
    TraceState t;
    __shared__ unsigned long long s_stack[SMEM_STACK * 128];
    unsigned long long stack_lo[STACK_DEPTH - SMEM_STACK];
    const HybridStack<SMEM_STACK> stack{s_stack + threadIdx.x, stack_lo};
    t.cur = ST_DONE;
    bool have = false, exhausted = false;
    uint32_t p = 0;
    int type = 0;
    for (;;) {
        if (HOME && have && t.cur == ST_DONE) {
            if (type == 0) {
                __stcs(&wf.cont[p].w, t.tmax);
                if (!t.found) __stcs(&wf.hit[p], make_uint4(TRB_MISS, 0u, 0u, 0u));
            } else if (type == 1) __stcs(&wf.shadow[p].w, __uint_as_float(t.found ? 1u : 0u));
            else {
                __stcs(&wf.mis[p].w, t.tmax);
                if (!t.found) __stcs(&wf.a[p].w, __uint_as_float(TRB_MISS));
            }
            have = false;
        } else if (have && t.cur == ST_DONE) {
            if (type == 0) {
                __stcs(&wf.cont[p], make_float4(t.wd.x, t.wd.y, t.wd.z, t.tmax));
                __stcs(&wf.hit[p], make_uint4(t.found ? t.h_inst : TRB_MISS, t.h_prim, __float_as_uint(t.h_b1), __float_as_uint(t.h_b2)));
            } else if (type == 1) {
                __stcs(&wf.shadow[p], make_float4(t.wd.x, t.wd.y, t.wd.z, __uint_as_float(t.found ? 1u : 0u)));
            } else {
                __stcs(&wf.mis[p], make_float4(t.wd.x, t.wd.y, t.wd.z, t.tmax));
                float4 a4 = __ldcs(&wf.a[p]);
                a4.w = __uint_as_float(t.found ? t.h_inst : TRB_MISS);
                __stcs(&wf.a[p], a4);
            }
            have = false;
        }
        const unsigned idle = __ballot_sync(0xffffffffu, !have);
        if (idle != 0 && !exhausted && (__popc(idle) >= WF_REFILL_IDLE || idle == 0xffffffffu)) {
            const int leader = __ffs(idle) - 1;
            uint32_t base = 0;
            if (lane == leader) base = atomicAdd(&cnt_r[WF_TRACE_HEAD], (uint32_t)__popc(idle));
            base = __shfl_sync(0xffffffffu, base, leader);
            if (base >= total) exhausted = true;
            else if (!have) {
                const uint32_t i = base + __popc(idle & lt_mask);
                if (i < total) {
                    if (q_sorted) { const uint32_t e = __ldg(&q_sorted[i]); type = (int)(e >> 30); p = e & WF_PATH_MASK; }
                    else if (i < n_cont) { type = 0; p = wf.q_cont[i]; }
                    else if (i < n_cont + n_shadow) { type = 1; p = wf.q_shadow[i - n_cont]; }
                    else { type = 2; p = wf.q_mis[i - n_cont - n_shadow]; }
                    const float4 o4 = __ldcs(&wf.org[p]);
                    const float4 d4 = __ldcs(type == 0 ? &wf.cont[p] : (type == 1 ? &wf.shadow[p] : &wf.mis[p]));
                    Ray ray; ray.o = mk(o4.x, o4.y, o4.z); ray.d = mk(d4.x, d4.y, d4.z);
                    ray.tmin = QUERY ? o4.w : ((type == 0 && round == 0) ? 0.0f : 0.001f);
                    ray.tmax = QUERY ? d4.w : (type == 1 ? 0.999f : finf());
                    trace_init(sc, t, ray, type == 1 && shadow_any, ANIM ? __ldg(&wf.thr[p].w) : 0.0f, QUADS && PHASED, (flags & WF_TRACE_FORCE_EXACT_BOX) != 0);
                    t.xf_row = wf_xf_row<ANIM>(wf, p);
                    if (PHASED) { stack.put(0, (unsigned long long)ST_DONE); t.sp = 1; }
                    if (HOME) {
                        const float4 lo = __ldg(&sc.tlas->root_lo), hi = __ldg(&sc.tlas->root_hi);
                        if (STATS) cnt.node++;
                        float te;
                        t.cur = box_hit(lo, hi, t.o, t.inv, (t.neg & 1u) != 0, (t.neg & 2u) != 0, (t.neg & 4u) != 0, t.tmin, t.tmax, te) ? __float_as_uint(lo.w) : ST_POP;
                    }
                    have = true;
                }
            }
        }
        const unsigned busy0 = __ballot_sync(0xffffffffu, have);
        if (busy0 == 0) { if (exhausted) break; else continue; }
        if (PHASED) {
            const int thr_o = (int)(sched & 255u);
            for (;;) {
#pragma unroll
                for (int k = 0; k < WF_BURST; ++k)
                    if (trace_is_node(t.cur)) {
                        if (PIPE != 0 && !QUADS) step_nodes2<STATS, (PIPE & 1) != 0>(t, stack, cnt, rp.error_flag);
                        else step_nodes<STATS, QUADS>(t, stack, cnt, rp.error_flag);
                    }
                const bool is_a = trace_is_node(t.cur), is_o = !is_a && t.cur != ST_DONE;
                const unsigned m_a = __ballot_sync(0xffffffffu, is_a), m_o = __ballot_sync(0xffffffffu, is_o);
                if ((m_a | m_o) == 0) break;
                if (!exhausted && 32 - __popc(m_a | m_o) >= WF_REFILL_IDLE) break;
                if (m_o != 0 && (m_a == 0 || __popc(m_o) >= thr_o)) {
                    if (is_o) {
                        const RayHome home{&wf.org[p], type == 0 ? &wf.cont[p] : (type == 1 ? &wf.shadow[p] : &wf.mis[p]), &wf.hit[p], &wf.a[p].w, type};
                        if ((t.cur & REF_TAG) == REF_LEAF && t.level_inst != TRB_MISS) step_triangle<STATS, HOME>(t, cnt, &home);
                        else step_other<STATS, ANIM, HOME>(sc, t, stack, cnt, &home);
                    }
                }
            }
        } else {
            for (;;) {
                if (have && t.cur != ST_DONE) trace_step<STATS, ANIM>(sc, t, stack, cnt, rp.error_flag);
                const unsigned running = __ballot_sync(0xffffffffu, have && t.cur != ST_DONE);
                if (running == 0) break;
                if (!exhausted && 32 - __popc(running) >= WF_REFILL_IDLE) break;
            }
        }
    }
    if (rp.stats) {
        if (STATS) {
            unsigned long long v[3] = {cnt.node, cnt.tri, cnt.inst};
            for (int k = 0; k < 3; ++k) {
                unsigned long long x = v[k];
                for (int o = 16; o > 0; o >>= 1) x += __shfl_xor_sync(0xffffffffu, x, o);
                if (lane == 0 && x) atomicAdd(&rp.stats->node_tests + k, x);
            }
        }
        if (blockIdx.x == 0 && threadIdx.x == 0) {
            atomicAdd(round == 0 ? &rp.stats->rays_primary : &rp.stats->rays_continuation, (unsigned long long)n_cont);
            atomicAdd(&rp.stats->rays_shadow, (unsigned long long)n_shadow);
            atomicAdd(&rp.stats->rays_mis, (unsigned long long)n_mis);
        }
    }
}

__device__ __forceinline__ void finish_sample(const DScene& sc, const RenderParams& rp, const WfState& wf, uint32_t p, f3 illum, int mode) {
    if (mode == 2) { wf.rad[p] = make_float4(illum.x, illum.y, illum.z, 1.0f); return; }
    const f3 c = mk(clampf(illum.x, 0.0f, 1.0f), clampf(illum.y, 0.0f, 1.0f), clampf(illum.z, 0.0f, 1.0f));
    if (mode == 0) wf.rad[p] = make_float4(c.x, c.y, c.z, 1.0f);
    else {
        const SampleId id = sample_id(sc, rp, p);
        const PixelStreams ps = pixel_streams(rp.seed, id.pixel);
        float sx, sy, tm;
        sample_position(rp, ps, id, sx, sy, tm);
        trb_sample* out = reinterpret_cast<trb_sample*>(rp.samples_out) + p;
        out->x = sx; out->y = sy; out->r = c.x; out->g = c.y; out->b = c.z;
    }
}
template <int MODE>
__device__ __forceinline__ uint32_t wf_flags(float4 o4, uint32_t round) { return (MODE == 2 && round == 0) ? 0u : __float_as_uint(o4.w); }
template <int MODE>
__device__ __forceinline__ uint32_t wf_stream(const DScene& sc, const RenderParams& rp, const WfState& wf, uint32_t p) {
    if (MODE == 2) return __float_as_uint(wf.illum[p].w);
    const SampleId id = sample_id(sc, rp, p);
    return rng_absorb(rng_absorb(rng_seed(rp.seed), id.pixel), id.si);
}

template <int MODE, bool ANIM, int MINB>
__global__ void __launch_bounds__(128, MINB) k_wf_shade(const __grid_constant__ DScene sc, const __grid_constant__ RenderParams rp, const __grid_constant__ WfState wf,
                                                   uint32_t round) {
    uint32_t* cnt_r = wf.counters + round * WF_CNT;
    uint32_t* cnt_n = wf.counters + (round + 1) * WF_CNT;
    const uint32_t n = cnt_r[WF_N_ACTIVE];
    const uint32_t* __restrict__ act = wf.q_active[round & 1];
    uint32_t* act_next = wf.q_active[(round + 1) & 1];
    uint32_t* ending_next = wf.q_ending[(round + 1) & 1];
    const int lane = threadIdx.x & 31;
    if (round > 0) {
        const uint32_t n_end = cnt_r[WF_N_ENDING];
        const uint32_t* __restrict__ ending = wf.q_ending[round & 1];
        for (;;) {
            uint32_t base = 0;
            if (lane == 0) base = atomicAdd(&cnt_r[WF_ENDING_HEAD], 32u);
            base = __shfl_sync(0xffffffffu, base, 0);
            if (base >= n_end) break;
            const uint32_t i = base + lane;
            if (i < n_end) {
                const uint32_t p = ending[i];
                const float4 o4 = wf.org[p];
                const uint32_t fl = __float_as_uint(o4.w);
                const float4 il4 = wf.illum[p];
                const float4 a4 = wf.a[p], b4 = wf.b[p], t4 = wf.tprev[p];
                bool occluded = false, mis_ok = false;
                if (fl & WF_F_SHADOW) occluded = __float_as_uint(wf.shadow[p].w) != 0u;
                if (fl & WF_F_MIS) {
                    const float4 m4 = wf.mis[p];
                    mis_ok = mis_sees_light<ANIM>(sc, mk(o4.x, o4.y, o4.z), mk(m4.x, m4.y, m4.z), __float_as_uint(b4.w), __float_as_uint(a4.w), m4.w, wf.thr[p].w, wf_xf_row<ANIM>(wf, p));
                }
                const f3 illum = mk(il4.x, il4.y, il4.z) + mk(t4.x, t4.y, t4.z) * direct_resolve(mk(a4.x, a4.y, a4.z), mk(b4.x, b4.y, b4.z), occluded, mis_ok);
                finish_sample(sc, rp, wf, p, illum, MODE);
            }
        }
    }
    for (;;) {
        uint32_t base = 0;
        if (lane == 0) base = atomicAdd(&cnt_r[WF_SHADE_HEAD], 32u);
        base = __shfl_sync(0xffffffffu, base, 0);
        if (base >= n) break;
        const uint32_t i = base + lane;
        const bool valid = i < n;
        uint32_t p = 0;
        bool push_cont = false, push_shadow = false, push_mis = false, push_active = false, push_ending = false;
        f3 new_org = splat(0.0f);
        if (valid) {
            p = round == 0 ? i : act[i];
            const float4 o4 = wf.org[p];
            const uint32_t fl = wf_flags<MODE>(o4, round);
            const f3 org = mk(o4.x, o4.y, o4.z);
            float4 il4 = wf.illum[p];
            f3 illum = mk(il4.x, il4.y, il4.z);
            bool done = false;
            const float4 th4 = wf.thr[p];
            const float time = th4.w;
            const float* xf_row = wf_xf_row<ANIM>(wf, p);
            if (round > 0) {
                const float4 a4 = wf.a[p], b4 = wf.b[p], t4 = wf.tprev[p];
                bool occluded = false, mis_ok = false;
                if (fl & WF_F_SHADOW) occluded = __float_as_uint(wf.shadow[p].w) != 0u;
                if (fl & WF_F_MIS) {
                    const float4 m4 = wf.mis[p];
                    mis_ok = mis_sees_light<ANIM>(sc, org, mk(m4.x, m4.y, m4.z), __float_as_uint(b4.w), __float_as_uint(a4.w), m4.w, time, xf_row);
                }
                illum = illum + mk(t4.x, t4.y, t4.z) * direct_resolve(mk(a4.x, a4.y, a4.z), mk(b4.x, b4.y, b4.z), occluded, mis_ok);
                done = (fl & WF_F_TERMINATE) != 0;
            }
            if (!done) {
                const float4 c4 = wf.cont[p];
                const uint4 h4 = wf.hit[p];
                if (h4.x == TRB_MISS) done = true;
                else {
                    Ray ray; ray.o = org; ray.d = mk(c4.x, c4.y, c4.z); ray.tmin = 0.0f; ray.tmax = c4.w;
                    HitRec h; h.t = c4.w; h.inst = h4.x; h.prim = h4.y; h.b1 = __uint_as_float(h4.z); h.b2 = __uint_as_float(h4.w);
                    Surf s;
                    surface_at<ANIM>(sc, ray, h, s, time, xf_row);
                    f3 first_ng;
                    if (round == 0) { first_ng = s.ng; wf.ng[p] = make_float4(s.ng.x, s.ng.y, s.ng.z, 0.0f); }
                    else { const float4 n4 = wf.ng[p]; first_ng = mk(n4.x, n4.y, n4.z); }
                    const uint32_t hs = MODE == 2 ? __float_as_uint(il4.w) : wf_stream<MODE>(sc, rp, wf, p);
                    BounceOut o;
                    shade_bounce<ANIM>(sc, s, h.inst, ray.d, first_ng, round, (fl & WF_F_SPECULAR) != 0, hs, mk(th4.x, th4.y, th4.z), time, illum, o, xf_row, rp.ld_offset);
                    const uint32_t nf = (o.specular ? WF_F_SPECULAR : 0u) | (o.terminate ? WF_F_TERMINATE : 0u) | (o.ds.has_shadow ? WF_F_SHADOW : 0u) |
                                        (o.ds.has_mis ? WF_F_MIS : 0u);
                    push_cont = !o.terminate; push_shadow = o.ds.has_shadow; push_mis = o.ds.has_mis;
                    push_active = push_cont || push_shadow || push_mis;
                    push_ending = push_active && o.terminate;
                    if (push_active) {
                        new_org = o.org;
                        wf.org[p] = make_float4(o.org.x, o.org.y, o.org.z, __uint_as_float(nf));
                        if (push_cont) wf.cont[p] = make_float4(o.next_d.x, o.next_d.y, o.next_d.z, finf());
                        if (push_shadow) wf.shadow[p] = make_float4(o.ds.shadow_d.x, o.ds.shadow_d.y, o.ds.shadow_d.z, 0.0f);
                        if (push_mis) wf.mis[p] = make_float4(o.ds.mis_d.x, o.ds.mis_d.y, o.ds.mis_d.z, finf());
                        wf.a[p] = make_float4(o.ds.a.x, o.ds.a.y, o.ds.a.z, __uint_as_float(TRB_MISS));
                        wf.b[p] = make_float4(o.ds.b.x, o.ds.b.y, o.ds.b.z, __uint_as_float(o.light));
                        wf.tprev[p] = make_float4(o.t_before.x, o.t_before.y, o.t_before.z, 0.0f);
                        wf.thr[p] = make_float4(o.throughput.x, o.throughput.y, o.throughput.z, time);
                        wf.illum[p] = make_float4(illum.x, illum.y, illum.z, MODE == 2 ? il4.w : 0.0f);
                    } else done = true;
                }
            }
            if (done && MODE == 2) finish_sample(sc, rp, wf, p, illum, MODE);
            else if (done) {
                const f3 c = mk(clampf(illum.x, 0.0f, 1.0f), clampf(illum.y, 0.0f, 1.0f), clampf(illum.z, 0.0f, 1.0f));
                if (MODE == 0) wf.rad[p] = make_float4(c.x, c.y, c.z, 1.0f);
                else {
                    const SampleId id = sample_id(sc, rp, p);
                    const PixelStreams ps = pixel_streams(rp.seed, id.pixel);
                    float sx, sy, tm;
                    sample_position(rp, ps, id, sx, sy, tm);
                    trb_sample* out = reinterpret_cast<trb_sample*>(rp.samples_out) + p;
                    out->x = sx; out->y = sy; out->r = c.x; out->g = c.y; out->b = c.z;
                }
            }
        }
        wf_push(wf.q_cont, &cnt_n[WF_N_CONT], push_cont, p);
        wf_push(wf.q_shadow, &cnt_n[WF_N_SHADOW], push_shadow, p);
        wf_push(wf.q_mis, &cnt_n[WF_N_MIS], push_mis, p);
        wf_push(act_next, &cnt_n[WF_N_ACTIVE], push_active && !push_ending, p);
        wf_push(ending_next, &cnt_n[WF_N_ENDING], push_ending, p);
        wf_bounds_add(wf.bounds + (round + 1) * 8, push_active, new_org);
    }
}

constexpr uint32_t S_WHITTED = 4096;
__device__ __forceinline__ void whitted_2d(uint32_t hs, uint32_t node, uint32_t slot, float& x, float& y) {
    x = ld_vdc(0, scramble_of(rng_absorb(hs, S_WHITTED + 8 * node + slot)));
    y = ld_sobol(0, scramble_of(rng_absorb(hs, S_WHITTED + 8 * node + slot + 1)));
}
__device__ __forceinline__ float whitted_1d(uint32_t hs, uint32_t node, uint32_t slot) { return ld_vdc(0, scramble_of(rng_absorb(hs, S_WHITTED + 8 * node + slot))); }

template <bool ANIM>
__device__ __noinline__ void light_sample_incident(const DScene& sc, uint32_t li, f3 p, float u0, float u1, float time, f3& lrad, f3& wi, float& pdf, f3& seg) {
    const DInstance& light = sc.instances[li];
    const uint32_t kind = __ldg(&light.kind), shape = __ldg(&light.shape);
    const float p0 = __ldg(&light.p0), p1 = __ldg(&light.p1);
    f3 emission;
    emission_at<ANIM>(sc, light, time, emission.x, emission.y, emission.z);
    float linv[16], lmat[16];
    instance_inv_mat<ANIM>(sc, light, time, linv, lmat);
    if (kind == TRB_INST_EMITTER_POINT) {
        const f3 pos = xf_point(lmat, splat(0.0f));
        wi = unit(pos - p);
        lrad = emission / len2(pos - p);
        pdf = 1.0f;
        seg = pos - p;
        return;
    }
    const f3 pl = xf_point(linv, p);
    f3 ps, nl;
    shape_sample(shape, p0, p1, pl, u0, u1, ps, nl);
    const f3 wil = unit(ps - pl);
    pdf = shape_pdf(shape, p0, p1, pl, wil);
    lrad = dot3(-wil, nl) > 0.0f ? emission : splat(0.0f);
    const f3 pw = xf_point(lmat, ps);
    wi = xf_vector(lmat, wil);
    seg = pw - p;
}

template <bool ANIM>
__device__ f3 whitted_illum(const DScene& sc, const Ray& ray, uint32_t depth, const HitRec& hit, uint32_t node, uint32_t hs, float time, bool ref_shadow,
                            RayCounts& rc, Cnt& cnt, int* err) {
    Surf s;
    surface_at<ANIM>(sc, ray, hit, s, time);
    const DInstance& in = sc.instances[hit.inst];
    Mat m;
    load_mat_at(sc, __ldg(&in.material), s.u, s.v, time, m);
    Frame fr;
    make_frame(s, fr);
    const f3 wo = -ray.d;
    float u0, u1;
    whitted_2d(hs, node, 0, u0, u1);
    f3 illum = splat(0.0f);
    if (depth == 0 && __ldg(&in.kind) != TRB_INST_RECEIVER) {
        if (dot3(-ray.d, s.ng) > 0.0f) { f3 le; emission_at<ANIM>(sc, in, time, le.x, le.y, le.z); illum = illum + le; }
        else illum = illum + splat(0.0f);
    }
    for (uint32_t k = 0; k < sc.n_lights; ++k) {
        f3 lrad, wi, seg; float pdf;
        light_sample_incident<ANIM>(sc, __ldg(&sc.lights[k]), s.p, u0, u1, time, lrad, wi, pdf, seg);
        const f3 f = bsdf_eval(sc, m, fr, wo, wi, BX_ALL);
        if (!black(lrad) && !black(f)) {
            Ray sr; sr.o = s.p; sr.d = seg; sr.tmin = 0.001f; sr.tmax = 0.999f;
            HitRec sh;
            rc.shadow++;
            if (!scene_trace<true, ANIM>(sc, sr, sh, !ref_shadow, cnt, err, time)) illum = illum + f * lrad * fabsf(dot3(wi, fr.n)) / pdf;
        }
    }
    if (depth < sc.max_depth) {
#pragma unroll 1
        for (int which = 0; which < 2; ++which) {
            const uint32_t flags = BX_SPECULAR | (which == 0 ? BX_REFLECTION : BX_TRANSMISSION), slot = which == 0 ? 2u : 5u;
            float v0, v1;
            whitted_2d(hs, node, slot, v0, v1);
            const float vc = whitted_1d(hs, node, slot + 2);
            f3 f, wi; float pdf; uint32_t sampled;
            bsdf_sample(sc, m, fr, wo, flags, v0, v1, vc, f, wi, pdf, sampled);
            f3 out = splat(0.0f);
            if (pdf > 0.0f && !black(f) && fabsf(dot3(wi, fr.n)) != 0.0f) {
                Ray r2; r2.o = fr.p; r2.d = wi; r2.tmin = 0.001f; r2.tmax = finf();
                HitRec h2;
                rc.cont++;
                if (scene_trace<true, ANIM>(sc, r2, h2, false, cnt, err, time)) {
                    const f3 li = whitted_illum<ANIM>(sc, r2, depth + 1, h2, 2 * node + (uint32_t)which, hs, time, ref_shadow, rc, cnt, err);
                    out = f * li * fabsf(dot3(wi, fr.n)) / pdf;
                }
            }
            illum = illum + out;
        }
    }
    return illum;
}

template <int MODE, bool ANIM>
__global__ void __launch_bounds__(128) k_simple_integrator(const __grid_constant__ DScene sc, const __grid_constant__ RenderParams rp, float4* rad, uint32_t n_paths,
                                                           uint32_t integrator, uint32_t flags, const trb_illum_ray* __restrict__ rays) {
    RayCounts rc = {0, 0, 0, 0};
    Cnt cnt = {0, 0, 0};
    uint32_t mine = 0;
    for (uint32_t p = blockIdx.x * blockDim.x + threadIdx.x; p < n_paths; p += gridDim.x * blockDim.x) {
        Ray ray;
        float time, sx = 0.0f, sy = 0.0f;
        uint32_t hpix, si;
        if (MODE == 2) {
            const trb_illum_ray& q = rays[p / rp.spp];
            ray.o = mk(q.o[0], q.o[1], q.o[2]); ray.d = mk(q.d[0], q.d[1], q.d[2]); ray.tmin = q.min_t; ray.tmax = q.max_t;
            time = q.time;
            hpix = rng_absorb(rng_seed(rp.seed), q.key); si = q.sample + p % rp.spp;
        } else {
            const SampleId id = sample_id(sc, rp, p);
            const PixelStreams ps = pixel_streams(rp.seed, id.pixel);
            hpix = ps.hpix; si = id.si;
            float tm;
            sample_position(rp, ps, id, sx, sy, tm);
            time = camera_ray<ANIM>(sc, sx, sy, tm, ray);
        }
        mine++; rc.primary++;
        HitRec hit;
        f3 c = splat(0.0f);
        if (scene_trace<true, ANIM>(sc, ray, hit, false, cnt, rp.error_flag, time)) {
            if (integrator == TRB_INTEGRATOR_NORMALS_DEBUG) {
                Surf s;
                surface_at<ANIM>(sc, ray, hit, s, time);
                Frame fr;
                make_frame(s, fr);
                c = (fr.n + splat(1.0f)) / 2.0f;
            } else c = whitted_illum<ANIM>(sc, ray, 0, hit, 1, rng_absorb(hpix, si), time, (flags & 4u) != 0, rc, cnt, rp.error_flag);
        }
        if (MODE == 2) { rad[p] = make_float4(c.x, c.y, c.z, 1.0f); continue; }
        c = mk(clampf(c.x, 0.0f, 1.0f), clampf(c.y, 0.0f, 1.0f), clampf(c.z, 0.0f, 1.0f));
        if (MODE == 0) rad[p] = make_float4(c.x, c.y, c.z, 1.0f);
        else { trb_sample* out = reinterpret_cast<trb_sample*>(rp.samples_out) + p; out->x = sx; out->y = sy; out->r = c.x; out->g = c.y; out->b = c.z; }
    }
    if (rp.stats) flush_stats(rp.stats, rc, cnt, mine, true);
}

__device__ __forceinline__ void load_frame(const WfState& wf, uint32_t p, Frame& fr, uint32_t& inst, float& u, float& v) {
    const float4 a = wf.f_p[p], n = wf.f_n[p], t = wf.f_t[p], b = wf.f_b[p];
    fr.p = mk(a.x, a.y, a.z); inst = __float_as_uint(a.w); u = n.w; v = t.w;
    fr.n = mk(n.x, n.y, n.z); fr.tan = mk(t.x, t.y, t.z); fr.bitan = mk(b.x, b.y, b.z);
}

template <int MODE, bool ANIM, int MINB>
__global__ void __launch_bounds__(128, MINB) k_wf_shade_a(const __grid_constant__ DScene sc, const __grid_constant__ RenderParams rp, const __grid_constant__ WfState wf,
                                                     uint32_t round) {
    uint32_t* cnt_r = wf.counters + round * WF_CNT;
    const uint32_t n = cnt_r[WF_N_ACTIVE];
    const uint32_t* __restrict__ act = wf.q_active[round & 1];
    const int lane = threadIdx.x & 31;
    for (;;) {
        uint32_t base = 0;
        if (lane == 0) base = atomicAdd(&cnt_r[WF_SHADE_HEAD], 32u);
        base = __shfl_sync(0xffffffffu, base, 0);
        if (base >= n) break;
        const uint32_t i = base + lane;
        uint32_t p = 0, mid_key = 0;
        bool push_mid = false;
        if (i < n) {
            p = round == 0 ? i : act[i];
            const float4 o4 = wf.org[p];
            const uint32_t fl = wf_flags<MODE>(o4, round);
            const f3 org = mk(o4.x, o4.y, o4.z);
            const float4 il4 = wf.illum[p];
            f3 illum = mk(il4.x, il4.y, il4.z);
            bool done = false;
            const float4 th4 = wf.thr[p];
            const float time = th4.w;
            const float* xf_row = wf_xf_row<ANIM>(wf, p);
            if (round > 0) {
                const float4 a4 = wf.a[p], b4 = wf.b[p], t4 = wf.tprev[p];
                bool occluded = false, mis_ok = false;
                if (fl & WF_F_SHADOW) occluded = __float_as_uint(wf.shadow[p].w) != 0u;
                if (fl & WF_F_MIS) {
                    const float4 m4 = wf.mis[p];
                    mis_ok = mis_sees_light<ANIM>(sc, org, mk(m4.x, m4.y, m4.z), __float_as_uint(b4.w), __float_as_uint(a4.w), m4.w, time, xf_row);
                }
                illum = illum + mk(t4.x, t4.y, t4.z) * direct_resolve(mk(a4.x, a4.y, a4.z), mk(b4.x, b4.y, b4.z), occluded, mis_ok);
                done = (fl & WF_F_TERMINATE) != 0;
            }
            if (!done) {
                const float4 c4 = wf.cont[p];
                const uint4 h4 = wf.hit[p];
                if (h4.x == TRB_MISS) done = true;
                else {
                    Ray ray; ray.o = org; ray.d = mk(c4.x, c4.y, c4.z); ray.tmin = 0.0f; ray.tmax = c4.w;
                    HitRec h; h.t = c4.w; h.inst = h4.x; h.prim = h4.y; h.b1 = __uint_as_float(h4.z); h.b2 = __uint_as_float(h4.w);
                    Surf s;
                    surface_at<ANIM>(sc, ray, h, s, time, xf_row);
                    f3 first_ng;
                    if (round == 0) { first_ng = s.ng; wf.ng[p] = make_float4(s.ng.x, s.ng.y, s.ng.z, 0.0f); }
                    else { const float4 n4 = wf.ng[p]; first_ng = mk(n4.x, n4.y, n4.z); }
                    bounce_emission<ANIM>(sc, h.inst, ray.d, first_ng, round, (fl & WF_F_SPECULAR) != 0, mk(th4.x, th4.y, th4.z), time, illum);
                    Frame fr;
                    make_frame(s, fr);
                    wf.f_p[p] = make_float4(fr.p.x, fr.p.y, fr.p.z, __uint_as_float(h.inst));
                    wf.f_n[p] = make_float4(fr.n.x, fr.n.y, fr.n.z, s.u);
                    wf.f_t[p] = make_float4(fr.tan.x, fr.tan.y, fr.tan.z, s.v);
                    wf.f_b[p] = make_float4(fr.bitan.x, fr.bitan.y, fr.bitan.z, 0.0f);
                    wf.illum[p] = make_float4(illum.x, illum.y, illum.z, MODE == 2 ? il4.w : 0.0f);
                    push_mid = true;
                    if (wf.mid_keyed) mid_key = __ldg(&sc.materials[__ldg(&sc.instances[h.inst].material)].type) & (WF_MID_BUCKETS - 1u);
                }
            }
            if (done) finish_sample(sc, rp, wf, p, illum, MODE);
        }
        wf_push_keyed(wf.q_mid, wf.n_paths, &cnt_r[WF_MID_K], push_mid, mid_key, p);
    }
}

template <bool ANIM, int MINB, int KIND = -1, int MODE = 0>
__global__ void __launch_bounds__(128, MINB) k_wf_shade_b(const __grid_constant__ DScene sc, const __grid_constant__ RenderParams rp, const __grid_constant__ WfState wf,
                                                     uint32_t round, uint32_t bucket_mask) {
    uint32_t* cnt_r = wf.counters + round * WF_CNT;
    uint32_t* cnt_n = wf.counters + (round + 1) * WF_CNT;
    const int lane = threadIdx.x & 31;
    for (uint32_t bucket = 0; bucket < WF_MID_BUCKETS; ++bucket) {
    if (!((bucket_mask >> bucket) & 1u)) continue;
    const uint32_t n = cnt_r[WF_MID_K + bucket];
    const uint32_t* __restrict__ q_mid = wf.q_mid + (size_t)bucket * wf.n_paths;
    for (;;) {
        if (n == 0) break;
        uint32_t base = 0;
        if (lane == 0) base = atomicAdd(&cnt_r[WF_B_HEAD_K + bucket], 32u);
        base = __shfl_sync(0xffffffffu, base, 0);
        if (base >= n) break;
        const uint32_t i = base + lane;
        uint32_t p = 0;
        bool push_shadow = false, push_mis = false;
        if (i < n) {
            p = q_mid[i];
            Frame fr; uint32_t inst; float tu, tv;
            load_frame(wf, p, fr, inst, tu, tv);
            const float4 c4 = wf.cont[p], th4 = wf.thr[p];
            const f3 wo = -mk(c4.x, c4.y, c4.z);
            Mat m;
            load_mat_at(sc, __ldg(&sc.instances[inst].material), tu, tv, th4.w, m);
            const uint32_t hs = wf_stream<MODE>(sc, rp, wf, p);
            DirectSetup ds; uint32_t light;
            bounce_direct<ANIM, KIND>(sc, m, fr, wo, round, hs, th4.w, ds, light, wf_xf_row<ANIM>(wf, p), rp.ld_offset);
            push_shadow = ds.has_shadow; push_mis = ds.has_mis;
            wf.org[p] = make_float4(fr.p.x, fr.p.y, fr.p.z, __uint_as_float((push_shadow ? WF_F_SHADOW : 0u) | (push_mis ? WF_F_MIS : 0u)));
            if (push_shadow) wf.shadow[p] = make_float4(ds.shadow_d.x, ds.shadow_d.y, ds.shadow_d.z, 0.0f);
            if (push_mis) wf.mis[p] = make_float4(ds.mis_d.x, ds.mis_d.y, ds.mis_d.z, finf());
            wf.a[p] = make_float4(ds.a.x, ds.a.y, ds.a.z, __uint_as_float(TRB_MISS));
            wf.b[p] = make_float4(ds.b.x, ds.b.y, ds.b.z, __uint_as_float(light));
            wf.tprev[p] = make_float4(th4.x, th4.y, th4.z, 0.0f);
        }
        wf_push(wf.q_shadow, &cnt_n[WF_N_SHADOW], push_shadow, p);
        wf_push(wf.q_mis, &cnt_n[WF_N_MIS], push_mis, p);
    }
    }
}

template <int MODE, bool ANIM, int MINB, int KIND = -1>
__global__ void __launch_bounds__(128, MINB) k_wf_shade_c(const __grid_constant__ DScene sc, const __grid_constant__ RenderParams rp, const __grid_constant__ WfState wf,
                                                     uint32_t round, uint32_t bucket_mask) {
    uint32_t* cnt_r = wf.counters + round * WF_CNT;
    uint32_t* cnt_n = wf.counters + (round + 1) * WF_CNT;
    uint32_t* act_next = wf.q_active[(round + 1) & 1];
    const int lane = threadIdx.x & 31;
    for (uint32_t bucket = 0; bucket < WF_MID_BUCKETS; ++bucket) {
    if (!((bucket_mask >> bucket) & 1u)) continue;
    const uint32_t n = cnt_r[WF_MID_K + bucket];
    const uint32_t* __restrict__ q_mid = wf.q_mid + (size_t)bucket * wf.n_paths;
    for (;;) {
        if (n == 0) break;
        uint32_t base = 0;
        if (lane == 0) base = atomicAdd(&cnt_r[WF_C_HEAD_K + bucket], 32u);
        base = __shfl_sync(0xffffffffu, base, 0);
        if (base >= n) break;
        const uint32_t i = base + lane;
        uint32_t p = 0;
        bool push_cont = false, push_active = false;
        f3 new_org = splat(0.0f);
        if (i < n) {
            p = q_mid[i];
            Frame fr; uint32_t inst; float tu, tv;
            load_frame(wf, p, fr, inst, tu, tv);
            const float4 c4 = wf.cont[p], th4 = wf.thr[p];
            const f3 wo = -mk(c4.x, c4.y, c4.z);
            Mat m;
            load_mat_at(sc, __ldg(&sc.instances[inst].material), tu, tv, th4.w, m);
            const uint32_t hs = wf_stream<MODE>(sc, rp, wf, p);
            ScatterOut so;
            bounce_scatter<KIND>(sc, m, fr, wo, round, hs, mk(th4.x, th4.y, th4.z), so, rp.ld_offset);
            const uint32_t fb = __float_as_uint(wf.org[p].w);
            push_cont = !so.terminate;
            push_active = push_cont || (fb & (WF_F_SHADOW | WF_F_MIS)) != 0u;
            if (push_active) {
                new_org = fr.p;
                wf.org[p] = make_float4(fr.p.x, fr.p.y, fr.p.z, __uint_as_float(fb | (so.specular ? WF_F_SPECULAR : 0u) | (so.terminate ? WF_F_TERMINATE : 0u)));
                if (push_cont) wf.cont[p] = make_float4(so.next_d.x, so.next_d.y, so.next_d.z, finf());
                wf.thr[p] = make_float4(so.throughput.x, so.throughput.y, so.throughput.z, th4.w);
            } else {
                const float4 il4 = wf.illum[p];
                finish_sample(sc, rp, wf, p, mk(il4.x, il4.y, il4.z), MODE);
            }
        }
        wf_push(wf.q_cont, &cnt_n[WF_N_CONT], push_cont, p);
        wf_push(act_next, &cnt_n[WF_N_ACTIVE], push_active, p);
        wf_bounds_add(wf.bounds + (round + 1) * 8, push_active, new_org);
    }
    }
}

template <bool ADAPT = false>
__global__ void __launch_bounds__(RENDER_THREADS) k_wf_film(const __grid_constant__ DScene sc, const __grid_constant__ RenderParams rp, const __grid_constant__ WfState wf) {
    extern __shared__ float4 tile[];
    __shared__ float s_table[256];
    const int T = 9 + 2 * max(sc.fpw_x, sc.fpw_y);
    for (int i = threadIdx.x; i < 256; i += RENDER_THREADS) s_table[i] = sc.filter_table[i];
    const uint32_t pix = threadIdx.x & 63, lane_s = threadIdx.x >> 6;
    uint32_t n_live = 0;
    if (ADAPT) n_live = ad_pass_blocks(rp);
    for (uint32_t item = blockIdx.x; item < (ADAPT ? n_live : rp.n_blocks); item += gridDim.x) {
        __syncthreads();
        for (int i = threadIdx.x; i < T * T; i += RENDER_THREADS) tile[i] = make_float4(0.f, 0.f, 0.f, 0.f);
        __syncthreads();
        const uint2 blk = rp.blocks[item];
        const uint32_t bx = blk.x * 8, by = blk.y * 8;
        SampleId id; id.item = item; id.pix = pix; id.px = bx + (pix & 7); id.py = by + (pix >> 3); id.pixel = id.py * sc.width + id.px;
        const PixelStreams ps = ADAPT ? pixel_streams_round(rp.seed, id.pixel, rp.ad_round) : pixel_streams(rp.seed, id.pixel);
        const bool on = !ADAPT || (rp.ad_state[id.pixel].x & trbh::AD_ACTIVE) != 0u;
        const int x_lo = max((int)bx - sc.fpw_x, 0), x_hi = min((int)bx + 8 + sc.fpw_x, (int)sc.width - 1);
        const int y_lo = max((int)by - sc.fpw_y, 0), y_hi = min((int)by + 8 + sc.fpw_y, (int)sc.height - 1);
        const int tx0 = (int)bx - sc.fpw_x, ty0 = (int)by - sc.fpw_y;
        for (uint32_t s = lane_s; on && s < rp.sample_count; s += 2) {
            id.si = rp.sample_first + s;
            float sx, sy, tm;
            if (ADAPT) sample_position_ad(rp, ps, id, sx, sy, tm);
            else sample_position(rp, ps, id, sx, sy, tm);
            const float4 c4 = wf.rad[((size_t)item * 64 + pix) * rp.sample_count + s];
            splat_sample(sc, tile, s_table, T, tx0, ty0, x_lo, x_hi, y_lo, y_hi, id.px, id.py, sx, sy, mk(c4.x, c4.y, c4.z));
        }
        __syncthreads();
        for (int i = threadIdx.x; i < T * T; i += RENDER_THREADS) {
            const int ix = tx0 + i % T, iy = ty0 + i / T;
            if (ix < x_lo || ix > x_hi || iy < y_lo || iy > y_hi) continue;
            const float4 v = tile[i];
            if (v.w == 0.0f && v.x == 0.0f && v.y == 0.0f && v.z == 0.0f) continue;
            float* dst = reinterpret_cast<float*>(rp.film + (size_t)iy * sc.width + ix);
            atomicAdd(dst + 0, v.x); atomicAdd(dst + 1, v.y); atomicAdd(dst + 2, v.z); atomicAdd(dst + 3, v.w);
        }
    }
}

template <bool ADAPT = false>
__global__ void __launch_bounds__(RENDER_THREADS) k_wf_film_v2(const __grid_constant__ DScene sc, const __grid_constant__ RenderParams rp, const __grid_constant__ WfState wf) {
    extern __shared__ float4 tiles[];
    __shared__ float s_table[256];
    const int T = 9 + 2 * max(sc.fpw_x, sc.fpw_y);
    for (int i = threadIdx.x; i < 256; i += RENDER_THREADS) s_table[i] = sc.filter_table[i];
    const uint32_t pix = threadIdx.x & 63, lane_s = threadIdx.x >> 6;
    float4* mine = tiles + (threadIdx.x >> 5) * (T * T);
    const int ry = (int)ceilf(sc.filter_h / sc.filter_inv_h) + 1, rx = (int)ceilf(sc.filter_w / sc.filter_inv_w) + 1;
    uint32_t n_live = 0;
    if (ADAPT) n_live = ad_pass_blocks(rp);
    for (uint32_t item = blockIdx.x; item < (ADAPT ? n_live : rp.n_blocks); item += gridDim.x) {
        __syncthreads();
        for (int i = threadIdx.x; i < 4 * T * T; i += RENDER_THREADS) tiles[i] = make_float4(0.f, 0.f, 0.f, 0.f);
        __syncthreads();
        const uint2 blk = rp.blocks[item];
        const uint32_t bx = blk.x * 8, by = blk.y * 8;
        SampleId id; id.item = item; id.pix = pix; id.px = bx + (pix & 7); id.py = by + (pix >> 3); id.pixel = id.py * sc.width + id.px;
        const PixelStreams ps = ADAPT ? pixel_streams_round(rp.seed, id.pixel, rp.ad_round) : pixel_streams(rp.seed, id.pixel);
        const bool on = !ADAPT || (rp.ad_state[id.pixel].x & trbh::AD_ACTIVE) != 0u;
        const int x_lo = max((int)bx - sc.fpw_x, 0), x_hi = min((int)bx + 8 + sc.fpw_x, (int)sc.width - 1);
        const int y_lo = max((int)by - sc.fpw_y, 0), y_hi = min((int)by + 8 + sc.fpw_y, (int)sc.height - 1);
        const int tx0 = (int)bx - sc.fpw_x, ty0 = (int)by - sc.fpw_y;
        for (uint32_t s = lane_s; s < rp.sample_count; s += 2) {
            id.si = rp.sample_first + s;
            float sx, sy, tm;
            if (ADAPT) sample_position_ad(rp, ps, id, sx, sy, tm);
            else sample_position(rp, ps, id, sx, sy, tm);
            const float4 c4 = on ? wf.rad[((size_t)item * 64 + pix) * rp.sample_count + s] : make_float4(0.f, 0.f, 0.f, 0.f);
            const float img_x = sx - 0.5f, img_y = sy - 0.5f;
            for (int dy = -ry; dy <= ry + 1; ++dy) {
                const int iy = (int)id.py + dy;
                const float fy = fabsf((float)iy - img_y) * sc.filter_inv_h;
                const bool vy = iy >= y_lo && iy <= y_hi && !(fy > sc.filter_h) &&
                                (!sc.film_block_filter || lock_block_takes(sy, iy, y_lo, y_hi, sc.fpw_y));
                const uint32_t fyi = min(f2u(fy * 16.0f), 15u);
                for (int dx = -rx; dx <= rx + 1; ++dx) {
                    const int ix = (int)id.px + dx;
                    const float fx = fabsf((float)ix - img_x) * sc.filter_inv_w;
                    if (on && vy && ix >= x_lo && ix <= x_hi && !(fx > sc.filter_w) && (!sc.film_block_filter || lock_block_takes(sx, ix, x_lo, x_hi, sc.fpw_x))) {
                        const uint32_t fxi = min(f2u(fx * 16.0f), 15u);
                        const float wgt = s_table[fyi * 16 + fxi];
                        float4* t = &mine[(iy - ty0) * T + (ix - tx0)];
                        float4 a = *t;
                        a.x += wgt * c4.x; a.y += wgt * c4.y; a.z += wgt * c4.z; a.w += wgt;
                        *t = a;
                    }
                    __syncwarp();
                }
            }
        }
        __syncthreads();
        for (int i = threadIdx.x; i < T * T; i += RENDER_THREADS) {
            const int ix = tx0 + i % T, iy = ty0 + i / T;
            if (ix < x_lo || ix > x_hi || iy < y_lo || iy > y_hi) continue;
            const float4 a = tiles[i], b = tiles[T * T + i], c = tiles[2 * T * T + i], d = tiles[3 * T * T + i];
            const float4 v = make_float4((a.x + b.x) + (c.x + d.x), (a.y + b.y) + (c.y + d.y), (a.z + b.z) + (c.z + d.z), (a.w + b.w) + (c.w + d.w));
            if (v.w == 0.0f && v.x == 0.0f && v.y == 0.0f && v.z == 0.0f) continue;
            float* dst = reinterpret_cast<float*>(rp.film + (size_t)iy * sc.width + ix);
            atomicAdd(dst + 0, v.x); atomicAdd(dst + 1, v.y); atomicAdd(dst + 2, v.z); atomicAdd(dst + 3, v.w);
        }
    }
}

template <bool ANIM>
__global__ void k_camera_rays(const __grid_constant__ DScene sc, const __grid_constant__ RenderParams rp, trb_ray* rays, float* xy) {
    const size_t n = (size_t)rp.n_blocks * 64 * rp.sample_count;
    for (size_t i = blockIdx.x * (size_t)blockDim.x + threadIdx.x; i < n; i += (size_t)gridDim.x * blockDim.x) {
        const uint32_t s = (uint32_t)(i % rp.sample_count), pix = (uint32_t)((i / rp.sample_count) % 64), item = (uint32_t)(i / ((size_t)64 * rp.sample_count));
        const uint2 blk = rp.blocks[item];
        const uint32_t px = blk.x * 8 + (pix & 7), py = blk.y * 8 + (pix >> 3);
        const PixelStreams ps = pixel_streams(rp.seed, py * sc.width + px);
        const uint32_t si = rp.sample_first + s;
        const uint32_t ip = permute_index(si, rp.spp, ps.kpos);
        const float sx = ld_vdc(ip, ps.scr0) + (float)px, sy = ld_sobol(ip, ps.scr1) + (float)py;
        const float tm = ld_vdc(permute_index(si, rp.spp, ps.ktime), ps.scrt);
        Ray r;
        camera_ray<ANIM>(sc, sx, sy, tm, r);
        rays[i].o[0] = r.o.x; rays[i].o[1] = r.o.y; rays[i].o[2] = r.o.z;
        rays[i].d[0] = r.d.x; rays[i].d[1] = r.d.y; rays[i].d[2] = r.d.z;
        rays[i].min_t = r.tmin; rays[i].max_t = r.tmax;
        xy[2 * i] = sx; xy[2 * i + 1] = sy;
    }
}

template <bool STATS, bool ANIM>
__global__ void __launch_bounds__(128) k_intersect(const __grid_constant__ DScene sc, size_t n, const trb_ray* __restrict__ rays, trb_hit* __restrict__ hits,
                                                    DStats* stats, int* err) {
    Cnt cnt = {0, 0, 0};
    RayCounts rc = {0, 0, 0, 0};
    for (size_t i = blockIdx.x * (size_t)blockDim.x + threadIdx.x; i < n; i += (size_t)gridDim.x * blockDim.x) {
        const float4 a = __ldg(reinterpret_cast<const float4*>(rays + i)), b = __ldg(reinterpret_cast<const float4*>(rays + i) + 1);
        Ray r; r.o = mk(a.x, a.y, a.z); r.d = mk(a.w, b.x, b.y); r.tmin = b.z; r.tmax = b.w;
        HitRec h;
        const bool hit = scene_trace<STATS, ANIM>(sc, r, h, false, cnt, err, sc.cam.shutter_open);
        rc.primary++;
        uint4 o; o.x = __float_as_uint(r.tmax); o.y = hit ? h.inst : TRB_MISS; o.z = hit ? h.prim : 0u; o.w = 0u;
        *reinterpret_cast<uint4*>(hits + i) = o;
    }
    if (stats) flush_stats(stats, rc, cnt, 0, STATS);
}

template <bool OCCLUSION>
__global__ void __launch_bounds__(256) k_query_load(const __grid_constant__ WfState wf, const trb_query_ray* __restrict__ rays) {
    const uint32_t n = wf.n_paths;
    for (uint32_t p = blockIdx.x * blockDim.x + threadIdx.x; p < n; p += gridDim.x * blockDim.x) {
        const float4* r = reinterpret_cast<const float4*>(rays + p);
        const float4 a = __ldg(r), b = __ldg(r + 1), c = __ldg(r + 2);
        wf.org[p] = make_float4(a.x, a.y, a.z, b.z);
        (OCCLUSION ? wf.shadow : wf.cont)[p] = make_float4(a.w, b.x, b.y, b.w);
        wf.thr[p] = make_float4(0.0f, 0.0f, 0.0f, c.x);
        (OCCLUSION ? wf.q_shadow : wf.q_cont)[p] = p;
    }
    if (blockIdx.x == 0 && threadIdx.x < WF_CNT) wf.counters[threadIdx.x] = threadIdx.x == (OCCLUSION ? WF_N_SHADOW : WF_N_CONT) ? n : 0u;
}
template <bool ANIM>
__global__ void __launch_bounds__(128) k_query_records(const __grid_constant__ DScene sc, const __grid_constant__ WfState wf, trb_intersection* __restrict__ out) {
    const uint32_t n = wf.n_paths;
    for (uint32_t p = blockIdx.x * blockDim.x + threadIdx.x; p < n; p += gridDim.x * blockDim.x) {
        const float4 o4 = wf.org[p], d4 = wf.cont[p];
        const uint4 h4 = wf.hit[p];
        float4 q[6] = {make_float4(d4.w, __uint_as_float(TRB_MISS), 0.0f, 0.0f), make_float4(0.0f, 0.0f, 0.0f, 0.0f), make_float4(0.0f, 0.0f, 0.0f, 0.0f),
                       make_float4(0.0f, 0.0f, 0.0f, 0.0f), make_float4(0.0f, 0.0f, 0.0f, 0.0f), make_float4(0.0f, 0.0f, 0.0f, 0.0f)};
        if (h4.x != TRB_MISS) {
            Ray ray; ray.o = mk(o4.x, o4.y, o4.z); ray.d = mk(d4.x, d4.y, d4.z); ray.tmin = o4.w; ray.tmax = d4.w;
            HitRec hit; hit.t = d4.w; hit.inst = h4.x; hit.prim = h4.y; hit.b1 = __uint_as_float(h4.z); hit.b2 = __uint_as_float(h4.w);
            const float time = wf.thr[p].w;
            Surf s;
            f3 dp_dv;
            surface_at<ANIM, true>(sc, ray, hit, s, time, wf_xf_row<ANIM>(wf, p), &dp_dv);
            const uint32_t material = __ldg(&sc.instances[hit.inst].material);
            q[0] = make_float4(d4.w, __uint_as_float(hit.inst), __uint_as_float(hit.prim), __uint_as_float(material));
            q[1] = make_float4(s.p.x, s.p.y, s.p.z, s.n.x);
            q[2] = make_float4(s.n.y, s.n.z, s.ng.x, s.ng.y);
            q[3] = make_float4(s.ng.z, s.u, s.v, time);
            q[4] = make_float4(s.dp_du.x, s.dp_du.y, s.dp_du.z, dp_dv.x);
            q[5] = make_float4(dp_dv.y, dp_dv.z, 0.0f, 0.0f);
        }
        float4* dst = reinterpret_cast<float4*>(out + p);
#pragma unroll
        for (int k = 0; k < 6; ++k) dst[k] = q[k];
    }
}
__global__ void __launch_bounds__(256) k_query_occluded(const __grid_constant__ WfState wf, uint8_t* __restrict__ out) {
    for (uint32_t p = blockIdx.x * blockDim.x + threadIdx.x; p < wf.n_paths; p += gridDim.x * blockDim.x) out[p] = __float_as_uint(wf.shadow[p].w) != 0u ? 1 : 0;
}

__global__ void __launch_bounds__(256) k_illum_load(const __grid_constant__ WfState wf, const trb_illum_ray* __restrict__ rays, uint32_t spp, uint32_t seed,
                                                    DStats* stats) {
    const uint32_t n = wf.n_paths, hseed = rng_seed(seed);
    for (uint32_t p = blockIdx.x * blockDim.x + threadIdx.x; p < n; p += gridDim.x * blockDim.x) {
        const float4* r = reinterpret_cast<const float4*>(rays + p / spp);
        const float4 a = __ldg(r), b = __ldg(r + 1), c = __ldg(r + 2);
        const uint32_t hs = rng_absorb(rng_absorb(hseed, __float_as_uint(c.y)), __float_as_uint(c.z) + p % spp);
        wf.org[p] = make_float4(a.x, a.y, a.z, b.z);
        wf.cont[p] = make_float4(a.w, b.x, b.y, b.w);
        wf.thr[p] = make_float4(1.0f, 1.0f, 1.0f, c.x);
        wf.illum[p] = make_float4(0.0f, 0.0f, 0.0f, __uint_as_float(hs));
        wf.q_cont[p] = p;
    }
    if (blockIdx.x == 0 && threadIdx.x == 0) {
        wf.counters[WF_N_ACTIVE] = n; wf.counters[WF_N_CONT] = n;
        if (stats) atomicAdd(&stats->camera_samples, (unsigned long long)n);
    }
    if (blockIdx.x == 0 && threadIdx.x < 64) {
        uint32_t* b = wf.bounds + threadIdx.x * 8;
        b[0] = b[1] = b[2] = b[3] = 0xffffffffu; b[4] = b[5] = b[6] = b[7] = 0u;
    }
}
__global__ void __launch_bounds__(128) k_illum_reduce(const float4* __restrict__ rad, uint32_t n_rays, uint32_t spp, uint32_t clamp, float* __restrict__ rgb) {
    for (uint32_t i = blockIdx.x * blockDim.x + threadIdx.x; i < n_rays; i += gridDim.x * blockDim.x) {
        const float4* r = rad + (size_t)i * spp;
        f3 sum = splat(0.0f);
        for (uint32_t j = 0; j < spp; ++j) {
            const float4 v = r[j];
            const f3 c = clamp ? mk(clampf(v.x, 0.0f, 1.0f), clampf(v.y, 0.0f, 1.0f), clampf(v.z, 0.0f, 1.0f)) : mk(v.x, v.y, v.z);
            sum = j == 0 ? c : sum + c;
        }
        const float k = (float)spp;
        rgb[3 * (size_t)i] = sum.x / k; rgb[3 * (size_t)i + 1] = sum.y / k; rgb[3 * (size_t)i + 2] = sum.z / k;
    }
}

__device__ __forceinline__ bool record_bsdf(const DScene& sc, uint32_t n_materials, const trb_intersection* rec, Mat& m, Frame& fr) {
    const float4* r = reinterpret_cast<const float4*>(rec);
    const float4 a = __ldg(r);
    if (__float_as_uint(a.y) == TRB_MISS || __float_as_uint(a.w) >= n_materials) return false;
    const float4 b = __ldg(r + 1), c = __ldg(r + 2), d = __ldg(r + 3), e = __ldg(r + 4);
    Surf s;
    s.p = mk(b.x, b.y, b.z); s.n = mk(b.w, c.x, c.y); s.ng = mk(c.z, c.w, d.x); s.u = d.y; s.v = d.z; s.dp_du = mk(e.x, e.y, e.z);
    load_mat_at(sc, __float_as_uint(a.w), d.y, d.z, d.w, m);
    make_frame(s, fr);
    return true;
}
__global__ void __launch_bounds__(128) k_bsdf_eval(const __grid_constant__ DScene sc, uint32_t n_materials, size_t n, const trb_intersection* __restrict__ rec,
                                                   const trb_bsdf_eval_query* __restrict__ q, float4* __restrict__ out) {
    for (size_t i = blockIdx.x * (size_t)blockDim.x + threadIdx.x; i < n; i += (size_t)gridDim.x * blockDim.x) {
        float4 o = make_float4(0.0f, 0.0f, 0.0f, 0.0f);
        Mat m; Frame fr;
        if (record_bsdf(sc, n_materials, rec + i, m, fr)) {
            const float4* qq = reinterpret_cast<const float4*>(q + i);
            const float4 a = __ldg(qq), b = __ldg(qq + 1);
            const f3 wo = mk(a.x, a.y, a.z), wi = mk(b.x, b.y, b.z);
            const uint32_t flags = __float_as_uint(a.w);
            const f3 f = bsdf_eval(sc, m, fr, wo, wi, flags);
            o = make_float4(f.x, f.y, f.z, bsdf_pdf(m, fr, wo, wi, flags));
        }
        out[i] = o;
    }
}
__global__ void __launch_bounds__(128) k_bsdf_sample(const __grid_constant__ DScene sc, uint32_t n_materials, size_t n, const trb_intersection* __restrict__ rec,
                                                     const trb_bsdf_sample_query* __restrict__ q, trb_bsdf_sample_result* __restrict__ out) {
    for (size_t i = blockIdx.x * (size_t)blockDim.x + threadIdx.x; i < n; i += (size_t)gridDim.x * blockDim.x) {
        float4 o0 = make_float4(0.0f, 0.0f, 0.0f, 0.0f), o1 = o0;
        Mat m; Frame fr;
        if (record_bsdf(sc, n_materials, rec + i, m, fr)) {
            const float4* qq = reinterpret_cast<const float4*>(q + i);
            const float4 a = __ldg(qq), b = __ldg(qq + 1);
            f3 f, wi; float pdf; uint32_t sampled;
            bsdf_sample(sc, m, fr, mk(a.x, a.y, a.z), __float_as_uint(a.w), b.x, b.y, b.z, f, wi, pdf, sampled);
            o0 = make_float4(f.x, f.y, f.z, pdf);
            o1 = make_float4(wi.x, wi.y, wi.z, __uint_as_float(sampled));
        }
        float4* dst = reinterpret_cast<float4*>(out + i);
        dst[0] = o0; dst[1] = o1;
    }
}
__device__ __forceinline__ bool is_light(const DScene& sc, uint32_t li) { return li < sc.n_instances && __ldg(&sc.instances[li].kind) != TRB_INST_RECEIVER; }
template <bool ANIM>
__global__ void __launch_bounds__(128) k_light_sample(const __grid_constant__ DScene sc, size_t n, const trb_light_query* __restrict__ q, trb_light_sample_result* __restrict__ out) {
    for (size_t i = blockIdx.x * (size_t)blockDim.x + threadIdx.x; i < n; i += (size_t)gridDim.x * blockDim.x) {
        const float4* qq = reinterpret_cast<const float4*>(q + i);
        const float4 a = __ldg(qq), b = __ldg(qq + 1);
        const uint32_t li = __float_as_uint(b.z);
        const float4 z = make_float4(0.0f, 0.0f, 0.0f, 0.0f);
        float4 o[5] = {z, z, z, z, z};
        if (is_light(sc, li)) {
            const f3 p = mk(a.x, a.y, a.z);
            f3 lrad, wi, seg; float pdf;
            light_sample_incident<ANIM>(sc, li, p, b.x, b.y, a.w, lrad, wi, pdf, seg);
            const uint32_t delta = __ldg(&sc.instances[li].kind) == TRB_INST_EMITTER_POINT ? 1u : 0u;
            o[0] = make_float4(lrad.x, lrad.y, lrad.z, pdf);
            o[1] = make_float4(wi.x, wi.y, wi.z, __uint_as_float(delta));
            o[2] = make_float4(p.x, p.y, p.z, seg.x);
            o[3] = make_float4(seg.y, seg.z, 0.001f, 0.999f);
            o[4] = make_float4(a.w, 0.0f, 0.0f, 0.0f);
        }
        float4* dst = reinterpret_cast<float4*>(out + i);
#pragma unroll
        for (int k = 0; k < 5; ++k) dst[k] = o[k];
    }
}
template <bool ANIM>
__device__ __noinline__ float light_pdf(const DScene& sc, uint32_t li, f3 p, f3 wi, float time) {
    const DInstance& light = sc.instances[li];
    if (__ldg(&light.kind) == TRB_INST_EMITTER_POINT) return 0.0f;
    float linv[16];
    instance_inv<ANIM>(sc, light, time, linv);
    const f3 pl = xf_point(linv, p);
    const f3 wl = unit(xf_vector(linv, wi));
    return shape_pdf(__ldg(&light.shape), __ldg(&light.p0), __ldg(&light.p1), pl, wl);
}
template <bool ANIM>
__global__ void __launch_bounds__(128) k_light_pdf(const __grid_constant__ DScene sc, size_t n, const trb_light_pdf_query* __restrict__ q, float* __restrict__ pdf) {
    for (size_t i = blockIdx.x * (size_t)blockDim.x + threadIdx.x; i < n; i += (size_t)gridDim.x * blockDim.x) {
        const float4* qq = reinterpret_cast<const float4*>(q + i);
        const float4 a = __ldg(qq), b = __ldg(qq + 1);
        const uint32_t li = __float_as_uint(b.w);
        pdf[i] = is_light(sc, li) ? light_pdf<ANIM>(sc, li, mk(a.x, a.y, a.z), mk(b.x, b.y, b.z), a.w) : 0.0f;
    }
}
template <bool ANIM>
__global__ void __launch_bounds__(128) k_emitted(const __grid_constant__ DScene sc, size_t n, const trb_emit_query* __restrict__ q, float* __restrict__ rgb) {
    for (size_t i = blockIdx.x * (size_t)blockDim.x + threadIdx.x; i < n; i += (size_t)gridDim.x * blockDim.x) {
        const float4* qq = reinterpret_cast<const float4*>(q + i);
        const float4 a = __ldg(qq), b = __ldg(qq + 1);
        const uint32_t inst = __float_as_uint(b.w);
        f3 le = splat(0.0f);
        if (is_light(sc, inst) && dot3(mk(a.x, a.y, a.z), mk(b.x, b.y, b.z)) > 0.0f) emission_at<ANIM>(sc, sc.instances[inst], a.w, le.x, le.y, le.z);
        rgb[3 * i] = le.x; rgb[3 * i + 1] = le.y; rgb[3 * i + 2] = le.z;
    }
}

struct FrameBuild {
    DInstance* instances;
    trbh::Box3* bounds;
    uint32_t n;
    float shutter_open, shutter_close;
    float* cx; float* cy; float* cz; uint32_t* idx; uint32_t* task; uint32_t* rec_of;
    trb_bvh_node* nodes; uint32_t* order; uint32_t* counts;
    DPair* pairs; DBvh* hdr;
};
__device__ __forceinline__ trbh::Box3 shape_bounds_dev(const DScene& sc, const DInstance& in) {
    trbh::Box3 b;
    const float p0 = in.p0, p1 = in.p1;
    switch (in.shape) {
        case TRB_SHAPE_SPHERE: for (int i = 0; i < 3; ++i) { b.lo[i] = -p0; b.hi[i] = p0; } break;
        case TRB_SHAPE_DISK: b.lo[0] = b.lo[1] = -p0; b.hi[0] = b.hi[1] = p0; b.lo[2] = -0.1f; b.hi[2] = 0.1f; break;
        case TRB_SHAPE_RECT: { const float hw = p0 / 2.0f, hh = p1 / 2.0f; b.lo[0] = -hw; b.lo[1] = -hh; b.hi[0] = hw; b.hi[1] = hh; b.lo[2] = b.hi[2] = 0.0f; break; }
        case TRB_SHAPE_MESH: { const DBvh& h = sc.meshes[in.mesh].bvh; b.lo[0] = h.root_lo.x; b.lo[1] = h.root_lo.y; b.lo[2] = h.root_lo.z; b.hi[0] = h.root_hi.x; b.hi[1] = h.root_hi.y; b.hi[2] = h.root_hi.z; break; }
        default: for (int i = 0; i < 3; ++i) b.lo[i] = b.hi[i] = 0.0f;
    }
    return b;
}
__global__ void __launch_bounds__(64) k_frame_instances(const __grid_constant__ DScene sc, const __grid_constant__ FrameBuild fb) {
    const uint32_t i = blockIdx.x * blockDim.x + threadIdx.x;
    if (i >= fb.n) return;
    DInstance& in = fb.instances[i];
    const uint32_t first = in.xf_first, cnt = in.xf_count;
    const trbh::Xf w = trbh::animated_xf(sc.splines, first, cnt, sc.keyframes, sc.knots, fb.shutter_open, sc.level_xf);
#pragma unroll
    for (int k = 0; k < 16; ++k) { in.inv[k] = w.inv.m[k]; in.mat[k] = w.fwd.m[k]; }
    const trbh::Box3 local = shape_bounds_dev(sc, in);
    trbh::Box3 acc;
    if (!trbh::xf_is_animated(sc.splines, first, cnt)) acc = trbh::arvo_bounds(w.fwd, local);
    else {
        acc = trbh::box_empty_hd();
        for (int k = 0; k < 128; ++k) {
            const float u = (float)k / 127.0f;
            const float time = fb.shutter_open * (1.0f - u) + fb.shutter_close * u;
            const trbh::Xf x = trbh::animated_xf(sc.splines, first, cnt, sc.keyframes, sc.knots, time, sc.level_xf);
            trbh::box_grow_hd(acc, trbh::arvo_bounds(x.fwd, local));
        }
    }
    fb.bounds[i] = acc;
}
__global__ void k_tlas_build(const __grid_constant__ FrameBuild fb) {
    if (blockIdx.x != 0 || threadIdx.x != 0) return;
    trbh::BvhBuildArrays B{fb.bounds, fb.n, 4u, fb.cx, fb.cy, fb.cz, fb.idx, fb.task, fb.nodes, fb.order, 0u, 0u};
    trbh::bvh_build_arrays(B);
    const trb_bvh_node* in = fb.nodes;
    uint32_t n_rec = 0;
    bool ok = true;
    for (uint32_t i = 0; i < B.n_nodes; ++i) if (!(in[i].b & TRB_BVH_LEAF)) fb.rec_of[i] = n_rec++;
    auto ref_of = [&](uint32_t i) -> uint32_t {
        if (in[i].b & TRB_BVH_LEAF) {
            const uint32_t cnt = in[i].b & ~TRB_BVH_LEAF, first = in[i].a;
            if (cnt > 31 || first >= (1u << 25)) ok = false;
            return REF_LEAF | (cnt << 25) | first;
        }
        return REF_INTERIOR | fb.rec_of[i];
    };
    for (uint32_t i = 0; i < B.n_nodes; ++i) {
        if (in[i].b & TRB_BVH_LEAF) continue;
        const trb_bvh_node& l = in[i + 1];
        const trb_bvh_node& r = in[in[i].a];
        DPair& p = fb.pairs[fb.rec_of[i]];
        p.l_lo = make_float4(l.bmin[0], l.bmin[1], l.bmin[2], __uint_as_float(ref_of(i + 1)));
        p.l_hi = make_float4(l.bmax[0], l.bmax[1], l.bmax[2], __uint_as_float(ref_of(in[i].a)));
        p.r_lo = make_float4(r.bmin[0], r.bmin[1], r.bmin[2], __uint_as_float(in[i].b));
        p.r_hi = make_float4(r.bmax[0], r.bmax[1], r.bmax[2], 0.f);
    }
    fb.hdr->pairs = fb.pairs;
    fb.hdr->root_lo = make_float4(in[0].bmin[0], in[0].bmin[1], in[0].bmin[2], __uint_as_float(ref_of(0)));
    fb.hdr->root_hi = make_float4(in[0].bmax[0], in[0].bmax[1], in[0].bmax[2], 0.f);
    fb.counts[0] = B.n_nodes; fb.counts[1] = B.n_order; fb.counts[2] = ok ? 1u : 0u;
}

__global__ void k_srgb8(size_t n, const float4* __restrict__ film, uint8_t* __restrict__ rgb8) {
    for (size_t i = blockIdx.x * (size_t)blockDim.x + threadIdx.x; i < n; i += (size_t)gridDim.x * blockDim.x) {
        const float4 c = film[i];
        uint8_t o[3] = {0, 0, 0};
        if (c.w > 0.0f) {
            const float v[3] = {c.x / c.w, c.y / c.w, c.z / c.w};
            for (int k = 0; k < 3; ++k) {
                const float x = clampf(v[k], 0.0f, 1.0f);
                const float s = x <= 0.0031308f ? 12.92f * x : (1.0f + 0.055f) * dpow(x, 1.0f / 2.4f) - 0.055f;
                const float q = s * 255.0f;
                o[k] = (uint8_t)f2u(q > 255.0f ? 255.0f : q);
            }
        }
        rgb8[3 * i] = o[0]; rgb8[3 * i + 1] = o[1]; rgb8[3 * i + 2] = o[2];
    }
}

template <bool ANIM>
__global__ void __launch_bounds__(256) k_wf_generate_ad(const __grid_constant__ DScene sc, const __grid_constant__ RenderParams rp, const __grid_constant__ WfState wf) {
    const uint32_t n = ad_pass_blocks(rp) * 64 * rp.sample_count;
    if (n == 0) return;
    const uint32_t lane = threadIdx.x & 31, stride = gridDim.x * blockDim.x;
    for (uint32_t p = blockIdx.x * blockDim.x + threadIdx.x; p - lane < n; p += stride) {
        bool on = false;
        if (p < n) {
            const SampleId id = sample_id(sc, rp, p);
            on = (rp.ad_state[id.pixel].x & trbh::AD_ACTIVE) != 0u;
            float time = 0.0f;
            if (on) {
                const PixelStreams ps = pixel_streams_round(rp.seed, id.pixel, rp.ad_round);
                float sx, sy, tm;
                sample_position_ad(rp, ps, id, sx, sy, tm);
                Ray ray;
                time = camera_ray<ANIM>(sc, sx, sy, tm, ray);
                wf.org[p] = make_float4(ray.o.x, ray.o.y, ray.o.z, __uint_as_float(0u));
                wf.cont[p] = make_float4(ray.d.x, ray.d.y, ray.d.z, finf());
            } else {
                wf.org[p] = make_float4(0.0f, 0.0f, 0.0f, __uint_as_float(0u));
                wf.cont[p] = make_float4(0.0f, 0.0f, 0.0f, finf());
                wf.hit[p] = make_uint4(TRB_MISS, 0u, 0u, 0u);
            }
            wf.thr[p] = make_float4(1.0f, 1.0f, 1.0f, time);
            wf.illum[p] = make_float4(0.0f, 0.0f, 0.0f, 0.0f);
        }
        const unsigned m = __ballot_sync(0xffffffffu, on);
        wf_push(wf.q_cont, &wf.counters[WF_N_CONT], on, p);
        if (lane == 0 && m && rp.stats) atomicAdd(&rp.stats->camera_samples, (unsigned long long)__popc(m));
    }
    if (blockIdx.x == 0 && threadIdx.x == 0) { wf.counters[WF_N_ACTIVE] = n; wf.counters[WF_N_PATHS] = n; }
    if (blockIdx.x == 0 && threadIdx.x < 64) {
        uint32_t* b = wf.bounds + threadIdx.x * 8;
        b[0] = b[1] = b[2] = b[3] = 0xffffffffu; b[4] = b[5] = b[6] = b[7] = 0u;
    }
}

__global__ void __launch_bounds__(128) k_ad_decide(const __grid_constant__ DScene sc, const __grid_constant__ RenderParams rp, const __grid_constant__ WfState wf,
                                                   uint32_t* block_flags) {
    trbh::AdSchedule sch;
    sch.min = rp.ad_min; sch.max = rp.ad_max; sch.step = rp.ad_step; sch.max_per_pixel = rp.ad_max_per_pixel; sch.rounds = 0;
    const uint32_t n = ad_pass_blocks(rp) * 64;
    for (uint32_t t = blockIdx.x * blockDim.x + threadIdx.x; t < n; t += gridDim.x * blockDim.x) {
        SampleId id;
        id.item = t >> 6; id.pix = t & 63;
        const uint2 blk = rp.blocks[id.item];
        id.px = blk.x * 8 + (id.pix & 7); id.py = blk.y * 8 + (id.pix >> 3); id.pixel = id.py * sc.width + id.px;
        const uint4 st4 = rp.ad_state[id.pixel];
        if (!(st4.x & trbh::AD_ACTIVE)) continue;
        trbh::AdPixel st; st.taken = st4.x; st.avg = __uint_as_float(st4.y); st.lmin = __uint_as_float(st4.z); st.lmax = __uint_as_float(st4.w);
        PixelStreams ps;
        if (rp.samples_out) ps = pixel_streams_round(rp.seed, id.pixel, rp.ad_round);
        for (uint32_t s = 0; s < rp.sample_count; ++s) {
            const float4 c = wf.rad[(size_t)t * rp.sample_count + s];
            const uint32_t slot = rp.sample_first + s;
            trbh::ad_add(st, slot, trbh::ad_luminance(c.x, c.y, c.z), rp.ad_round == 0);
            if (rp.samples_out) {
                id.si = slot;
                float sx, sy, tm;
                sample_position_ad(rp, ps, id, sx, sy, tm);
                trb_sample* out = reinterpret_cast<trb_sample*>(rp.samples_out) + ((size_t)rp.ad_block_index[id.item] * 64 + id.pix) * rp.ad_max_per_pixel + slot;
                out->x = sx; out->y = sy; out->r = c.x; out->g = c.y; out->b = c.z;
            }
        }
        const bool more = trbh::ad_finish(st, sch, rp.ad_round);
        rp.ad_state[id.pixel] = make_uint4(st.taken, __float_as_uint(st.avg), __float_as_uint(st.lmin), __float_as_uint(st.lmax));
        if (more) block_flags[id.item] = 1u;
    }
}

__global__ void k_ad_init(const __grid_constant__ DScene sc, const uint2* blocks, uint32_t n_blocks, uint4* state, uint2* list, uint32_t* list_index,
                          uint32_t* list_count) {
    if (blockIdx.x == 0 && threadIdx.x == 0) *list_count = n_blocks;
    for (uint32_t t = blockIdx.x * blockDim.x + threadIdx.x; t < n_blocks * 64; t += gridDim.x * blockDim.x) {
        const uint2 blk = blocks[t >> 6];
        const uint32_t pixel = (blk.y * 8 + ((t & 63) >> 3)) * sc.width + blk.x * 8 + (t & 7);
        const trbh::AdPixel p = trbh::ad_initial();
        state[pixel] = make_uint4(p.taken, __float_as_uint(p.avg), __float_as_uint(p.lmin), __float_as_uint(p.lmax));
        if ((t & 63) == 0) { list[t >> 6] = blk; list_index[t >> 6] = t >> 6; }
    }
}

__global__ void __launch_bounds__(1024) k_ad_compact(uint32_t* flags, const uint32_t* in_count, const uint2* in_list, const uint32_t* in_index,
                                                     uint2* out_list, uint32_t* out_index, uint32_t* out_count) {
    __shared__ uint32_t part[1024];
    __shared__ uint32_t base;
    const uint32_t n = *in_count;
    if (threadIdx.x == 0) base = 0;
    for (uint32_t c0 = 0; c0 < n; c0 += 1024) {
        const uint32_t i = c0 + threadIdx.x;
        const uint32_t f = i < n && flags[i] ? 1u : 0u;
        __syncthreads();
        part[threadIdx.x] = f;
        __syncthreads();
        for (uint32_t s = 1; s < 1024; s <<= 1) {
            const uint32_t v = threadIdx.x >= s ? part[threadIdx.x - s] : 0u;
            __syncthreads();
            part[threadIdx.x] += v;
            __syncthreads();
        }
        if (f) { const uint32_t o = base + part[threadIdx.x] - 1u; out_list[o] = in_list[i]; out_index[o] = in_index[i]; }
        if (i < n) flags[i] = 0u;
        __syncthreads();
        if (threadIdx.x == 1023) base += part[1023];
    }
    __syncthreads();
    if (threadIdx.x == 0) *out_count = base;
}

__global__ void k_ad_pixel_spp(const __grid_constant__ DScene sc, const uint2* blocks, uint32_t n_blocks, const uint4* state, uint32_t* spp) {
    for (uint32_t t = blockIdx.x * blockDim.x + threadIdx.x; t < n_blocks * 64; t += gridDim.x * blockDim.x) {
        const uint2 blk = blocks[t >> 6];
        const uint32_t pixel = (blk.y * 8 + ((t & 63) >> 3)) * sc.width + blk.x * 8 + (t & 7);
        spp[pixel] = state[pixel].x & ~trbh::AD_ACTIVE;
    }
}

__global__ void k_film_keys(uint32_t n, const uint32_t* __restrict__ regions, uint32_t n_regions, uint32_t* __restrict__ keys,
                            uint32_t* __restrict__ order) {
    for (uint32_t i = blockIdx.x * blockDim.x + threadIdx.x; i < n; i += gridDim.x * blockDim.x) {
        const uint32_t r = regions[i];
        keys[i] = r < n_regions ? r : n_regions;
        order[i] = i;
    }
}

__global__ void k_film_starts(uint32_t n, const uint32_t* __restrict__ keys, uint32_t n_regions, uint32_t* __restrict__ start) {
    for (uint32_t r = blockIdx.x * blockDim.x + threadIdx.x; r <= n_regions; r += gridDim.x * blockDim.x) {
        uint32_t lo = 0, hi = n;
        while (lo < hi) {
            const uint32_t mid = lo + (hi - lo) / 2;
            if (keys[mid] < r) lo = mid + 1; else hi = mid;
        }
        start[r] = lo;
    }
}

__device__ __forceinline__ uint32_t morton_block(uint32_t x, uint32_t y) {
    auto part = [](uint32_t v) {
        v &= 0x0000ffffu; v = (v ^ (v << 8)) & 0x00ff00ffu; v = (v ^ (v << 4)) & 0x0f0f0f0fu;
        v = (v ^ (v << 2)) & 0x33333333u; return (v ^ (v << 1)) & 0x55555555u;
    };
    return (part(y) << 1) + part(x);
}

constexpr int FILM_WRITE_THREADS = 64;
constexpr int FILM_CHUNK = 512;

__global__ void __launch_bounds__(FILM_WRITE_THREADS) k_film_gather(const __grid_constant__ DScene sc, const trb_sample* __restrict__ samples,
                                                                    const uint32_t* __restrict__ order, const uint32_t* __restrict__ start,
                                                                    float* __restrict__ film) {
    __shared__ float s_table[256];
    __shared__ float s_x[FILM_CHUNK], s_y[FILM_CHUNK], s_r[FILM_CHUNK], s_g[FILM_CHUNK], s_b[FILM_CHUNK];
    __shared__ uint32_t s_cand[16], s_code[16];
    __shared__ int s_ncand;
    const uint32_t nbx = sc.width / 8, nby = sc.height / 8;
    const uint32_t tbx = blockIdx.x % nbx, tby = blockIdx.x / nbx;
    for (int i = threadIdx.x; i < 256; i += FILM_WRITE_THREADS) s_table[i] = sc.filter_table[i];
    if (threadIdx.x == 0) {
        int nc = 0;
        const uint32_t bx0 = (uint32_t)max((int)tbx - (8 + sc.fpw_x) / 8, 0), bx1 = min(tbx + (uint32_t)(7 + sc.fpw_x) / 8, nbx - 1);
        const uint32_t by0 = (uint32_t)max((int)tby - (8 + sc.fpw_y) / 8, 0), by1 = min(tby + (uint32_t)(7 + sc.fpw_y) / 8, nby - 1);
        for (uint32_t by = by0; by <= by1; ++by)
            for (uint32_t bx = bx0; bx <= bx1; ++bx) {
                const uint32_t r = by * nbx + bx;
                if (start[r + 1] == start[r]) continue;
                const uint32_t code = morton_block(bx, by);
                int k = nc++;
                for (; k > 0 && s_code[k - 1] > code; --k) { s_code[k] = s_code[k - 1]; s_cand[k] = s_cand[k - 1]; }
                s_code[k] = code; s_cand[k] = r;
            }
        s_ncand = nc;
    }
    __syncthreads();
    const int ix = (int)(tbx * 8 + (threadIdx.x & 7)), iy = (int)(tby * 8 + (threadIdx.x >> 3));
    float* px = film + ((size_t)iy * sc.width + ix) * 4;
    float f0 = px[0], f1 = px[1], f2 = px[2], f3v = px[3];
    bool touched = false;
    const int nc = s_ncand;
    for (int c = 0; c < nc; ++c) {
        const uint32_t r = s_cand[c];
        const int rx = (int)(r % nbx) * 8, ry = (int)(r / nbx) * 8;
        const int x_lo = max(rx - sc.fpw_x, 0), x_hi = min(rx + 8 + sc.fpw_x, (int)sc.width - 1);
        const int y_lo = max(ry - sc.fpw_y, 0), y_hi = min(ry + 8 + sc.fpw_y, (int)sc.height - 1);
        const bool in = ix >= x_lo && ix <= x_hi && iy >= y_lo && iy <= y_hi;
        float a0 = 0.0f, a1 = 0.0f, a2 = 0.0f, a3 = 0.0f;
        const uint32_t s0 = start[r], s1 = start[r + 1];
        for (uint32_t b = s0; b < s1; b += FILM_CHUNK) {
            const uint32_t cnt = min(s1 - b, (uint32_t)FILM_CHUNK);
            __syncthreads();
            for (uint32_t j = threadIdx.x; j < cnt; j += FILM_WRITE_THREADS) {
                const trb_sample* sp = samples + order[b + j];
                s_x[j] = sp->x; s_y[j] = sp->y; s_r[j] = sp->r; s_g[j] = sp->g; s_b[j] = sp->b;
            }
            __syncthreads();
            if (!in) continue;
            for (uint32_t j = 0; j < cnt; ++j) {
                const float sx = s_x[j], sy = s_y[j];
                if (!lock_block_takes(sx, ix, x_lo, x_hi, sc.fpw_x) || !lock_block_takes(sy, iy, y_lo, y_hi, sc.fpw_y)) continue;
                const float fy = fabsf((float)iy - (sy - 0.5f)) * sc.filter_inv_h;
                if (fy > sc.filter_h) continue;
                const float fx = fabsf((float)ix - (sx - 0.5f)) * sc.filter_inv_w;
                if (fx > sc.filter_w) continue;
                const uint32_t fyi = min(f2u(fy * 16.0f), 15u), fxi = min(f2u(fx * 16.0f), 15u);
                const float wgt = s_table[fyi * 16 + fxi];
                a0 += wgt * s_r[j];
                a1 += wgt * s_g[j];
                a2 += wgt * s_b[j];
                a3 += wgt;
            }
        }
        if (in) { f0 += a0; f1 += a1; f2 += a2; f3v += a3; touched = true; }
    }
    if (touched) { px[0] = f0; px[1] = f1; px[2] = f2; px[3] = f3v; }
}

}
```

Before: 752.9.

## Interleave wavefront path-state arrays into paired AoS buffers

Merges separate per-path float4 arrays (org/cont, b/tprev, thr/illum, and the four frame arrays) into interleaved buffers so that fields read together sit in adjacent memory. This targets scattered loads on sorted or queued path indices, where each separate array touched costs its own cache line. The trade-off is that kernels touching only one field of a pair, such as trace reading only org or thr.w, now pull in a neighbouring field they do not need, and coalescing for sequentially indexed accesses drops.

```diff
diff --git a/tray_rust_b200/csrc/trb_api.cu b/tray_rust_b200/csrc/trb_api.cu
--- a/tray_rust_b200/csrc/trb_api.cu
+++ b/tray_rust_b200/csrc/trb_api.cu
@@ -402,8 +402,11 @@
         if (err == cudaSuccess) s->wf_allocs.push_back(*out);
     };
     trb::WfState& w = s->wf;
-    float4** f4[] = {&w.org, &w.cont, &w.shadow, &w.mis, &w.a, &w.b, &w.tprev, &w.thr, &w.illum, &w.ng, &w.rad, &w.f_p, &w.f_n, &w.f_t, &w.f_b};
+    float4** f4[] = {&w.shadow, &w.mis, &w.a, &w.ng, &w.rad};
     for (float4** q : f4) grab(cap * sizeof(float4), reinterpret_cast<void**>(q));
+    float4** f4x2[] = {&w.oc, &w.bt, &w.ti};
+    for (float4** q : f4x2) grab(cap * 2 * sizeof(float4), reinterpret_cast<void**>(q));
+    grab(cap * 4 * sizeof(float4), reinterpret_cast<void**>(&w.frame));
     grab(cap * sizeof(uint4), reinterpret_cast<void**>(&w.hit));
     uint32_t** u1[] = {&w.q_active[0], &w.q_active[1], &w.q_ending[0], &w.q_ending[1], &w.q_cont, &w.q_shadow, &w.q_mis};
     for (uint32_t** q : u1) grab(cap * sizeof(uint32_t), reinterpret_cast<void**>(q));
diff --git a/tray_rust_b200/csrc/trb_kernels.cuh b/tray_rust_b200/csrc/trb_kernels.cuh
--- a/tray_rust_b200/csrc/trb_kernels.cuh
+++ b/tray_rust_b200/csrc/trb_kernels.cuh
@@ -1574,16 +1574,13 @@
 }
 
 struct WfState {
-    float4* org;
-    float4* cont;
+    float4* oc;
     uint4* hit;
     float4* shadow;
     float4* mis;
     float4* a;
-    float4* b;
-    float4* tprev;
-    float4* thr;
-    float4* illum;
+    float4* bt;
+    float4* ti;
     float4* ng;
     float4* rad;
     uint32_t* q_active[2];
@@ -1596,15 +1593,19 @@
     uint32_t* sort_rank;
     uint32_t* sort_hist;
     uint32_t* sort_offs;
-    float4* f_p;
-    float4* f_n;
-    float4* f_t;
-    float4* f_b;
+    float4* frame;
     uint32_t* q_mid;
     uint32_t mid_keyed;
     float* xf_tab;
     uint32_t n_anim;
     uint32_t* bounds;
+
+    __device__ __forceinline__ float4& org(uint32_t p) const { return oc[2 * (size_t)p]; }
+    __device__ __forceinline__ float4& cont(uint32_t p) const { return oc[2 * (size_t)p + 1]; }
+    __device__ __forceinline__ float4& b(uint32_t p) const { return bt[2 * (size_t)p]; }
+    __device__ __forceinline__ float4& tprev(uint32_t p) const { return bt[2 * (size_t)p + 1]; }
+    __device__ __forceinline__ float4& thr(uint32_t p) const { return ti[2 * (size_t)p]; }
+    __device__ __forceinline__ float4& illum(uint32_t p) const { return ti[2 * (size_t)p + 1]; }
 };
 constexpr uint32_t WF_PATH_MASK = 0x3fffffffu;
 constexpr int WF_SORT_MAX_BITS = 6;
@@ -1686,7 +1687,7 @@
         const uint32_t p = (uint32_t)(i / wf.n_anim), k = (uint32_t)(i % wf.n_anim);
         const DInstance& in = sc.instances[__ldg(&sc.anim_instances[k])];
         float inv[16], mat[16];
-        eval_anim_xf(sc, __ldg(&in.spline_first), __ldg(&in.n_splines), wf.thr[p].w, inv, mat);
+        eval_anim_xf(sc, __ldg(&in.spline_first), __ldg(&in.n_splines), wf.thr(p).w, inv, mat);
         float4* dst = reinterpret_cast<float4*>(wf.xf_tab + i * 32);
 #pragma unroll
         for (int q = 0; q < 4; ++q) dst[q] = make_float4(inv[4 * q], inv[4 * q + 1], inv[4 * q + 2], inv[4 * q + 3]);
@@ -1705,7 +1706,7 @@
         for (uint32_t i = threadIdx.x; i < np * nu; i += blockDim.x) {
             const uint32_t lp = i / nu, u = i % nu;
             const trb_spline& sp = sc.splines[__ldg(&sc.uniq_splines[u])];
-            const float time = wf.thr[p0 + lp].w;
+            const float time = wf.thr(p0 + lp).w;
             const float lo = sc.knots[sp.knot_first + sp.degree], hi = sc.knots[sp.knot_first + sp.n_knots - 1 - sp.degree];
             const trbh::Xf t = trbh::keyframe_xf(trbh::spline_point(sp, sc.keyframes, sc.knots, trbh::clampf_hd(time, lo, hi)));
             float* dst = s_lvl + (size_t)i * 32;
@@ -1777,8 +1778,8 @@
     const uint32_t cmax = (1u << bits) - 1u, nb = 8u << (3u * bits);
     for (uint32_t i = blockIdx.x * blockDim.x + threadIdx.x; i < total; i += gridDim.x * blockDim.x) {
         const RayRef r = wf_ray_ref(wf, i, n_cont, n_shadow);
-        const float4 o4 = wf.org[r.p];
-        const float4 d4 = r.type == 0 ? wf.cont[r.p] : (r.type == 1 ? wf.shadow[r.p] : wf.mis[r.p]);
+        const float4 o4 = wf.org(r.p);
+        const float4 d4 = r.type == 0 ? wf.cont(r.p) : (r.type == 1 ? wf.shadow[r.p] : wf.mis[r.p]);
         const uint32_t cx = min(cmax, __float2uint_rz(fmaxf(0.0f, (o4.x - lo.x) * sx))), cy = min(cmax, __float2uint_rz(fmaxf(0.0f, (o4.y - lo.y) * sy))),
                        cz = min(cmax, __float2uint_rz(fmaxf(0.0f, (o4.z - lo.z) * sz)));
         const uint32_t m = spread3(cx) | (spread3(cy) << 1) | (spread3(cz) << 2);
@@ -1823,10 +1824,10 @@
         sample_position(rp, ps, id, sx, sy, tm);
         Ray ray;
         const float time = camera_ray<ANIM>(sc, sx, sy, tm, ray);
-        wf.org[p] = make_float4(ray.o.x, ray.o.y, ray.o.z, __uint_as_float(0u));
-        wf.cont[p] = make_float4(ray.d.x, ray.d.y, ray.d.z, finf());
-        wf.thr[p] = make_float4(1.0f, 1.0f, 1.0f, time);
-        wf.illum[p] = make_float4(0.0f, 0.0f, 0.0f, 0.0f);
+        wf.org(p) = make_float4(ray.o.x, ray.o.y, ray.o.z, __uint_as_float(0u));
+        wf.cont(p) = make_float4(ray.d.x, ray.d.y, ray.d.z, finf());
+        wf.thr(p) = make_float4(1.0f, 1.0f, 1.0f, time);
+        wf.illum(p) = make_float4(0.0f, 0.0f, 0.0f, 0.0f);
         wf.q_cont[p] = p;
     }
     if (blockIdx.x == 0 && threadIdx.x == 0) {
@@ -1862,7 +1863,7 @@
     for (;;) {
         if (HOME && have && t.cur == ST_DONE) {
             if (type == 0) {
-                __stcs(&wf.cont[p].w, t.tmax);
+                __stcs(&wf.cont(p).w, t.tmax);
                 if (!t.found) __stcs(&wf.hit[p], make_uint4(TRB_MISS, 0u, 0u, 0u));
             } else if (type == 1) __stcs(&wf.shadow[p].w, __uint_as_float(t.found ? 1u : 0u));
             else {
@@ -1872,7 +1873,7 @@
             have = false;
         } else if (have && t.cur == ST_DONE) {
             if (type == 0) {
-                __stcs(&wf.cont[p], make_float4(t.wd.x, t.wd.y, t.wd.z, t.tmax));
+                __stcs(&wf.cont(p), make_float4(t.wd.x, t.wd.y, t.wd.z, t.tmax));
                 __stcs(&wf.hit[p], make_uint4(t.found ? t.h_inst : TRB_MISS, t.h_prim, __float_as_uint(t.h_b1), __float_as_uint(t.h_b2)));
             } else if (type == 1) {
                 __stcs(&wf.shadow[p], make_float4(t.wd.x, t.wd.y, t.wd.z, __uint_as_float(t.found ? 1u : 0u)));
@@ -1898,12 +1899,12 @@
                     else if (i < n_cont) { type = 0; p = wf.q_cont[i]; }
                     else if (i < n_cont + n_shadow) { type = 1; p = wf.q_shadow[i - n_cont]; }
                     else { type = 2; p = wf.q_mis[i - n_cont - n_shadow]; }
-                    const float4 o4 = __ldcs(&wf.org[p]);
-                    const float4 d4 = __ldcs(type == 0 ? &wf.cont[p] : (type == 1 ? &wf.shadow[p] : &wf.mis[p]));
+                    const float4 o4 = __ldcs(&wf.org(p));
+                    const float4 d4 = __ldcs(type == 0 ? &wf.cont(p) : (type == 1 ? &wf.shadow[p] : &wf.mis[p]));
                     Ray ray; ray.o = mk(o4.x, o4.y, o4.z); ray.d = mk(d4.x, d4.y, d4.z);
                     ray.tmin = QUERY ? o4.w : ((type == 0 && round == 0) ? 0.0f : 0.001f);
                     ray.tmax = QUERY ? d4.w : (type == 1 ? 0.999f : finf());
-                    trace_init(sc, t, ray, type == 1 && shadow_any, ANIM ? __ldg(&wf.thr[p].w) : 0.0f, QUADS && PHASED, (flags & WF_TRACE_FORCE_EXACT_BOX) != 0);
+                    trace_init(sc, t, ray, type == 1 && shadow_any, ANIM ? __ldg(&wf.thr(p).w) : 0.0f, QUADS && PHASED, (flags & WF_TRACE_FORCE_EXACT_BOX) != 0);
                     t.xf_row = wf_xf_row<ANIM>(wf, p);
                     if (PHASED) { stack.put(0, (unsigned long long)ST_DONE); t.sp = 1; }
                     if (HOME) {
@@ -1933,7 +1934,7 @@
                 if (!exhausted && 32 - __popc(m_a | m_o) >= WF_REFILL_IDLE) break;
                 if (m_o != 0 && (m_a == 0 || __popc(m_o) >= thr_o)) {
                     if (is_o) {
-                        const RayHome home{&wf.org[p], type == 0 ? &wf.cont[p] : (type == 1 ? &wf.shadow[p] : &wf.mis[p]), &wf.hit[p], &wf.a[p].w, type};
+                        const RayHome home{&wf.org(p), type == 0 ? &wf.cont(p) : (type == 1 ? &wf.shadow[p] : &wf.mis[p]), &wf.hit[p], &wf.a[p].w, type};
                         if ((t.cur & REF_TAG) == REF_LEAF && t.level_inst != TRB_MISS) step_triangle<STATS, HOME>(t, cnt, &home);
                         else step_other<STATS, ANIM, HOME>(sc, t, stack, cnt, &home);
                     }
@@ -1982,7 +1983,7 @@
 __device__ __forceinline__ uint32_t wf_flags(float4 o4, uint32_t round) { return (MODE == 2 && round == 0) ? 0u : __float_as_uint(o4.w); }
 template <int MODE>
 __device__ __forceinline__ uint32_t wf_stream(const DScene& sc, const RenderParams& rp, const WfState& wf, uint32_t p) {
-    if (MODE == 2) return __float_as_uint(wf.illum[p].w);
+    if (MODE == 2) return __float_as_uint(wf.illum(p).w);
     const SampleId id = sample_id(sc, rp, p);
     return rng_absorb(rng_absorb(rng_seed(rp.seed), id.pixel), id.si);
 }
@@ -2008,15 +2009,15 @@
             const uint32_t i = base + lane;
             if (i < n_end) {
                 const uint32_t p = ending[i];
-                const float4 o4 = wf.org[p];
+                const float4 o4 = wf.org(p);
                 const uint32_t fl = __float_as_uint(o4.w);
-                const float4 il4 = wf.illum[p];
-                const float4 a4 = wf.a[p], b4 = wf.b[p], t4 = wf.tprev[p];
+                const float4 il4 = wf.illum(p);
+                const float4 a4 = wf.a[p], b4 = wf.b(p), t4 = wf.tprev(p);
                 bool occluded = false, mis_ok = false;
                 if (fl & WF_F_SHADOW) occluded = __float_as_uint(wf.shadow[p].w) != 0u;
                 if (fl & WF_F_MIS) {
                     const float4 m4 = wf.mis[p];
-                    mis_ok = mis_sees_light<ANIM>(sc, mk(o4.x, o4.y, o4.z), mk(m4.x, m4.y, m4.z), __float_as_uint(b4.w), __float_as_uint(a4.w), m4.w, wf.thr[p].w, wf_xf_row<ANIM>(wf, p));
+                    mis_ok = mis_sees_light<ANIM>(sc, mk(o4.x, o4.y, o4.z), mk(m4.x, m4.y, m4.z), __float_as_uint(b4.w), __float_as_uint(a4.w), m4.w, wf.thr(p).w, wf_xf_row<ANIM>(wf, p));
                 }
                 const f3 illum = mk(il4.x, il4.y, il4.z) + mk(t4.x, t4.y, t4.z) * direct_resolve(mk(a4.x, a4.y, a4.z), mk(b4.x, b4.y, b4.z), occluded, mis_ok);
                 finish_sample(sc, rp, wf, p, illum, MODE);
@@ -2035,17 +2036,17 @@
         f3 new_org = splat(0.0f);
         if (valid) {
             p = round == 0 ? i : act[i];
-            const float4 o4 = wf.org[p];
+            const float4 o4 = wf.org(p);
             const uint32_t fl = wf_flags<MODE>(o4, round);
             const f3 org = mk(o4.x, o4.y, o4.z);
-            float4 il4 = wf.illum[p];
+            float4 il4 = wf.illum(p);
             f3 illum = mk(il4.x, il4.y, il4.z);
             bool done = false;
-            const float4 th4 = wf.thr[p];
+            const float4 th4 = wf.thr(p);
             const float time = th4.w;
             const float* xf_row = wf_xf_row<ANIM>(wf, p);
             if (round > 0) {
-                const float4 a4 = wf.a[p], b4 = wf.b[p], t4 = wf.tprev[p];
+                const float4 a4 = wf.a[p], b4 = wf.b(p), t4 = wf.tprev(p);
                 bool occluded = false, mis_ok = false;
                 if (fl & WF_F_SHADOW) occluded = __float_as_uint(wf.shadow[p].w) != 0u;
                 if (fl & WF_F_MIS) {
@@ -2056,7 +2057,7 @@
                 done = (fl & WF_F_TERMINATE) != 0;
             }
             if (!done) {
-                const float4 c4 = wf.cont[p];
+                const float4 c4 = wf.cont(p);
                 const uint4 h4 = wf.hit[p];
                 if (h4.x == TRB_MISS) done = true;
                 else {
@@ -2077,15 +2078,15 @@
                     push_ending = push_active && o.terminate;
                     if (push_active) {
                         new_org = o.org;
-                        wf.org[p] = make_float4(o.org.x, o.org.y, o.org.z, __uint_as_float(nf));
-                        if (push_cont) wf.cont[p] = make_float4(o.next_d.x, o.next_d.y, o.next_d.z, finf());
+                        wf.org(p) = make_float4(o.org.x, o.org.y, o.org.z, __uint_as_float(nf));
+                        if (push_cont) wf.cont(p) = make_float4(o.next_d.x, o.next_d.y, o.next_d.z, finf());
                         if (push_shadow) wf.shadow[p] = make_float4(o.ds.shadow_d.x, o.ds.shadow_d.y, o.ds.shadow_d.z, 0.0f);
                         if (push_mis) wf.mis[p] = make_float4(o.ds.mis_d.x, o.ds.mis_d.y, o.ds.mis_d.z, finf());
                         wf.a[p] = make_float4(o.ds.a.x, o.ds.a.y, o.ds.a.z, __uint_as_float(TRB_MISS));
-                        wf.b[p] = make_float4(o.ds.b.x, o.ds.b.y, o.ds.b.z, __uint_as_float(o.light));
-                        wf.tprev[p] = make_float4(o.t_before.x, o.t_before.y, o.t_before.z, 0.0f);
-                        wf.thr[p] = make_float4(o.throughput.x, o.throughput.y, o.throughput.z, time);
-                        wf.illum[p] = make_float4(illum.x, illum.y, illum.z, MODE == 2 ? il4.w : 0.0f);
+                        wf.b(p) = make_float4(o.ds.b.x, o.ds.b.y, o.ds.b.z, __uint_as_float(o.light));
+                        wf.tprev(p) = make_float4(o.t_before.x, o.t_before.y, o.t_before.z, 0.0f);
+                        wf.thr(p) = make_float4(o.throughput.x, o.throughput.y, o.throughput.z, time);
+                        wf.illum(p) = make_float4(illum.x, illum.y, illum.z, MODE == 2 ? il4.w : 0.0f);
                     } else done = true;
                 }
             }
@@ -2245,7 +2246,8 @@
 }
 
 __device__ __forceinline__ void load_frame(const WfState& wf, uint32_t p, Frame& fr, uint32_t& inst, float& u, float& v) {
-    const float4 a = wf.f_p[p], n = wf.f_n[p], t = wf.f_t[p], b = wf.f_b[p];
+    const float4* f = wf.frame + 4 * (size_t)p;
+    const float4 a = f[0], n = f[1], t = f[2], b = f[3];
     fr.p = mk(a.x, a.y, a.z); inst = __float_as_uint(a.w); u = n.w; v = t.w;
     fr.n = mk(n.x, n.y, n.z); fr.tan = mk(t.x, t.y, t.z); fr.bitan = mk(b.x, b.y, b.z);
 }
@@ -2267,17 +2269,17 @@
         bool push_mid = false;
         if (i < n) {
             p = round == 0 ? i : act[i];
-            const float4 o4 = wf.org[p];
+            const float4 o4 = wf.org(p);
             const uint32_t fl = wf_flags<MODE>(o4, round);
             const f3 org = mk(o4.x, o4.y, o4.z);
-            const float4 il4 = wf.illum[p];
+            const float4 il4 = wf.illum(p);
             f3 illum = mk(il4.x, il4.y, il4.z);
             bool done = false;
-            const float4 th4 = wf.thr[p];
+            const float4 th4 = wf.thr(p);
             const float time = th4.w;
             const float* xf_row = wf_xf_row<ANIM>(wf, p);
             if (round > 0) {
-                const float4 a4 = wf.a[p], b4 = wf.b[p], t4 = wf.tprev[p];
+                const float4 a4 = wf.a[p], b4 = wf.b(p), t4 = wf.tprev(p);
                 bool occluded = false, mis_ok = false;
                 if (fl & WF_F_SHADOW) occluded = __float_as_uint(wf.shadow[p].w) != 0u;
                 if (fl & WF_F_MIS) {
@@ -2288,7 +2290,7 @@
                 done = (fl & WF_F_TERMINATE) != 0;
             }
             if (!done) {
-                const float4 c4 = wf.cont[p];
+                const float4 c4 = wf.cont(p);
                 const uint4 h4 = wf.hit[p];
                 if (h4.x == TRB_MISS) done = true;
                 else {
@@ -2302,11 +2304,12 @@
                     bounce_emission<ANIM>(sc, h.inst, ray.d, first_ng, round, (fl & WF_F_SPECULAR) != 0, mk(th4.x, th4.y, th4.z), time, illum);
                     Frame fr;
                     make_frame(s, fr);
-                    wf.f_p[p] = make_float4(fr.p.x, fr.p.y, fr.p.z, __uint_as_float(h.inst));
-                    wf.f_n[p] = make_float4(fr.n.x, fr.n.y, fr.n.z, s.u);
-                    wf.f_t[p] = make_float4(fr.tan.x, fr.tan.y, fr.tan.z, s.v);
-                    wf.f_b[p] = make_float4(fr.bitan.x, fr.bitan.y, fr.bitan.z, 0.0f);
-                    wf.illum[p] = make_float4(illum.x, illum.y, illum.z, MODE == 2 ? il4.w : 0.0f);
+                    float4* f = wf.frame + 4 * (size_t)p;
+                    f[0] = make_float4(fr.p.x, fr.p.y, fr.p.z, __uint_as_float(h.inst));
+                    f[1] = make_float4(fr.n.x, fr.n.y, fr.n.z, s.u);
+                    f[2] = make_float4(fr.tan.x, fr.tan.y, fr.tan.z, s.v);
+                    f[3] = make_float4(fr.bitan.x, fr.bitan.y, fr.bitan.z, 0.0f);
+                    wf.illum(p) = make_float4(illum.x, illum.y, illum.z, MODE == 2 ? il4.w : 0.0f);
                     push_mid = true;
                     if (wf.mid_keyed) mid_key = __ldg(&sc.materials[__ldg(&sc.instances[h.inst].material)].type) & (WF_MID_BUCKETS - 1u);
                 }
@@ -2340,7 +2343,7 @@
             p = q_mid[i];
             Frame fr; uint32_t inst; float tu, tv;
             load_frame(wf, p, fr, inst, tu, tv);
-            const float4 c4 = wf.cont[p], th4 = wf.thr[p];
+            const float4 c4 = wf.cont(p), th4 = wf.thr(p);
             const f3 wo = -mk(c4.x, c4.y, c4.z);
             Mat m;
             load_mat_at(sc, __ldg(&sc.instances[inst].material), tu, tv, th4.w, m);
@@ -2348,12 +2351,12 @@
             DirectSetup ds; uint32_t light;
             bounce_direct<ANIM, KIND>(sc, m, fr, wo, round, hs, th4.w, ds, light, wf_xf_row<ANIM>(wf, p), rp.ld_offset);
             push_shadow = ds.has_shadow; push_mis = ds.has_mis;
-            wf.org[p] = make_float4(fr.p.x, fr.p.y, fr.p.z, __uint_as_float((push_shadow ? WF_F_SHADOW : 0u) | (push_mis ? WF_F_MIS : 0u)));
+            wf.org(p) = make_float4(fr.p.x, fr.p.y, fr.p.z, __uint_as_float((push_shadow ? WF_F_SHADOW : 0u) | (push_mis ? WF_F_MIS : 0u)));
             if (push_shadow) wf.shadow[p] = make_float4(ds.shadow_d.x, ds.shadow_d.y, ds.shadow_d.z, 0.0f);
             if (push_mis) wf.mis[p] = make_float4(ds.mis_d.x, ds.mis_d.y, ds.mis_d.z, finf());
             wf.a[p] = make_float4(ds.a.x, ds.a.y, ds.a.z, __uint_as_float(TRB_MISS));
-            wf.b[p] = make_float4(ds.b.x, ds.b.y, ds.b.z, __uint_as_float(light));
-            wf.tprev[p] = make_float4(th4.x, th4.y, th4.z, 0.0f);
+            wf.b(p) = make_float4(ds.b.x, ds.b.y, ds.b.z, __uint_as_float(light));
+            wf.tprev(p) = make_float4(th4.x, th4.y, th4.z, 0.0f);
         }
         wf_push(wf.q_shadow, &cnt_n[WF_N_SHADOW], push_shadow, p);
         wf_push(wf.q_mis, &cnt_n[WF_N_MIS], push_mis, p);
@@ -2386,23 +2389,23 @@
             p = q_mid[i];
             Frame fr; uint32_t inst; float tu, tv;
             load_frame(wf, p, fr, inst, tu, tv);
-            const float4 c4 = wf.cont[p], th4 = wf.thr[p];
+            const float4 c4 = wf.cont(p), th4 = wf.thr(p);
             const f3 wo = -mk(c4.x, c4.y, c4.z);
             Mat m;
             load_mat_at(sc, __ldg(&sc.instances[inst].material), tu, tv, th4.w, m);
             const uint32_t hs = wf_stream<MODE>(sc, rp, wf, p);
             ScatterOut so;
             bounce_scatter<KIND>(sc, m, fr, wo, round, hs, mk(th4.x, th4.y, th4.z), so, rp.ld_offset);
-            const uint32_t fb = __float_as_uint(wf.org[p].w);
+            const uint32_t fb = __float_as_uint(wf.org(p).w);
             push_cont = !so.terminate;
             push_active = push_cont || (fb & (WF_F_SHADOW | WF_F_MIS)) != 0u;
             if (push_active) {
                 new_org = fr.p;
-                wf.org[p] = make_float4(fr.p.x, fr.p.y, fr.p.z, __uint_as_float(fb | (so.specular ? WF_F_SPECULAR : 0u) | (so.terminate ? WF_F_TERMINATE : 0u)));
-                if (push_cont) wf.cont[p] = make_float4(so.next_d.x, so.next_d.y, so.next_d.z, finf());
-                wf.thr[p] = make_float4(so.throughput.x, so.throughput.y, so.throughput.z, th4.w);
+                wf.org(p) = make_float4(fr.p.x, fr.p.y, fr.p.z, __uint_as_float(fb | (so.specular ? WF_F_SPECULAR : 0u) | (so.terminate ? WF_F_TERMINATE : 0u)));
+                if (push_cont) wf.cont(p) = make_float4(so.next_d.x, so.next_d.y, so.next_d.z, finf());
+                wf.thr(p) = make_float4(so.throughput.x, so.throughput.y, so.throughput.z, th4.w);
             } else {
-                const float4 il4 = wf.illum[p];
+                const float4 il4 = wf.illum(p);
                 finish_sample(sc, rp, wf, p, mk(il4.x, il4.y, il4.z), MODE);
             }
         }
@@ -2562,9 +2565,9 @@
     for (uint32_t p = blockIdx.x * blockDim.x + threadIdx.x; p < n; p += gridDim.x * blockDim.x) {
         const float4* r = reinterpret_cast<const float4*>(rays + p);
         const float4 a = __ldg(r), b = __ldg(r + 1), c = __ldg(r + 2);
-        wf.org[p] = make_float4(a.x, a.y, a.z, b.z);
-        (OCCLUSION ? wf.shadow : wf.cont)[p] = make_float4(a.w, b.x, b.y, b.w);
-        wf.thr[p] = make_float4(0.0f, 0.0f, 0.0f, c.x);
+        wf.org(p) = make_float4(a.x, a.y, a.z, b.z);
+        (OCCLUSION ? wf.shadow[p] : wf.cont(p)) = make_float4(a.w, b.x, b.y, b.w);
+        wf.thr(p) = make_float4(0.0f, 0.0f, 0.0f, c.x);
         (OCCLUSION ? wf.q_shadow : wf.q_cont)[p] = p;
     }
     if (blockIdx.x == 0 && threadIdx.x < WF_CNT) wf.counters[threadIdx.x] = threadIdx.x == (OCCLUSION ? WF_N_SHADOW : WF_N_CONT) ? n : 0u;
@@ -2573,14 +2576,14 @@
 __global__ void __launch_bounds__(128) k_query_records(const __grid_constant__ DScene sc, const __grid_constant__ WfState wf, trb_intersection* __restrict__ out) {
     const uint32_t n = wf.n_paths;
     for (uint32_t p = blockIdx.x * blockDim.x + threadIdx.x; p < n; p += gridDim.x * blockDim.x) {
-        const float4 o4 = wf.org[p], d4 = wf.cont[p];
+        const float4 o4 = wf.org(p), d4 = wf.cont(p);
         const uint4 h4 = wf.hit[p];
         float4 q[6] = {make_float4(d4.w, __uint_as_float(TRB_MISS), 0.0f, 0.0f), make_float4(0.0f, 0.0f, 0.0f, 0.0f), make_float4(0.0f, 0.0f, 0.0f, 0.0f),
                        make_float4(0.0f, 0.0f, 0.0f, 0.0f), make_float4(0.0f, 0.0f, 0.0f, 0.0f), make_float4(0.0f, 0.0f, 0.0f, 0.0f)};
         if (h4.x != TRB_MISS) {
             Ray ray; ray.o = mk(o4.x, o4.y, o4.z); ray.d = mk(d4.x, d4.y, d4.z); ray.tmin = o4.w; ray.tmax = d4.w;
             HitRec hit; hit.t = d4.w; hit.inst = h4.x; hit.prim = h4.y; hit.b1 = __uint_as_float(h4.z); hit.b2 = __uint_as_float(h4.w);
-            const float time = wf.thr[p].w;
+            const float time = wf.thr(p).w;
             Surf s;
             f3 dp_dv;
             surface_at<ANIM, true>(sc, ray, hit, s, time, wf_xf_row<ANIM>(wf, p), &dp_dv);
@@ -2608,10 +2611,10 @@
         const float4* r = reinterpret_cast<const float4*>(rays + p / spp);
         const float4 a = __ldg(r), b = __ldg(r + 1), c = __ldg(r + 2);
         const uint32_t hs = rng_absorb(rng_absorb(hseed, __float_as_uint(c.y)), __float_as_uint(c.z) + p % spp);
-        wf.org[p] = make_float4(a.x, a.y, a.z, b.z);
-        wf.cont[p] = make_float4(a.w, b.x, b.y, b.w);
-        wf.thr[p] = make_float4(1.0f, 1.0f, 1.0f, c.x);
-        wf.illum[p] = make_float4(0.0f, 0.0f, 0.0f, __uint_as_float(hs));
+        wf.org(p) = make_float4(a.x, a.y, a.z, b.z);
+        wf.cont(p) = make_float4(a.w, b.x, b.y, b.w);
+        wf.thr(p) = make_float4(1.0f, 1.0f, 1.0f, c.x);
+        wf.illum(p) = make_float4(0.0f, 0.0f, 0.0f, __uint_as_float(hs));
         wf.q_cont[p] = p;
     }
     if (blockIdx.x == 0 && threadIdx.x == 0) {
@@ -2846,15 +2849,15 @@
                 sample_position_ad(rp, ps, id, sx, sy, tm);
                 Ray ray;
                 time = camera_ray<ANIM>(sc, sx, sy, tm, ray);
-                wf.org[p] = make_float4(ray.o.x, ray.o.y, ray.o.z, __uint_as_float(0u));
-                wf.cont[p] = make_float4(ray.d.x, ray.d.y, ray.d.z, finf());
+                wf.org(p) = make_float4(ray.o.x, ray.o.y, ray.o.z, __uint_as_float(0u));
+                wf.cont(p) = make_float4(ray.d.x, ray.d.y, ray.d.z, finf());
             } else {
-                wf.org[p] = make_float4(0.0f, 0.0f, 0.0f, __uint_as_float(0u));
-                wf.cont[p] = make_float4(0.0f, 0.0f, 0.0f, finf());
+                wf.org(p) = make_float4(0.0f, 0.0f, 0.0f, __uint_as_float(0u));
+                wf.cont(p) = make_float4(0.0f, 0.0f, 0.0f, finf());
                 wf.hit[p] = make_uint4(TRB_MISS, 0u, 0u, 0u);
             }
-            wf.thr[p] = make_float4(1.0f, 1.0f, 1.0f, time);
-            wf.illum[p] = make_float4(0.0f, 0.0f, 0.0f, 0.0f);
+            wf.thr(p) = make_float4(1.0f, 1.0f, 1.0f, time);
+            wf.illum(p) = make_float4(0.0f, 0.0f, 0.0f, 0.0f);
         }
         const unsigned m = __ballot_sync(0xffffffffu, on);
         wf_push(wf.q_cont, &wf.counters[WF_N_CONT], on, p);
```

Result: faster. 768.4, median of 6 (+2.1%).
